# PetropoulakisPanagiotis/ICP-Variants

Hardware: AMD Instinct MI355X
Metric: ICP iterations/s (k-NN + point-to-plane linear, 370k-point ETH-Apartment-like pair) (higher is better)
Workload: dtype f32

## Files before the change

### icp-variants_amd/csrc/dev_bvh.hpp

```cpp
#ifndef ICP_ISEL_NATURAL
#define ICP_ISEL_NATURAL 0
#endif
#ifndef ICP_PRUNE_SLACK
#define ICP_PRUNE_SLACK 1.001f
#endif
constexpr int BVH_LEAF = 8;
#ifndef ICP_BVH_THREADS
#define ICP_BVH_THREADS 256
#endif
constexpr int BVH_THREADS = ICP_BVH_THREADS;
#ifndef ICP_QUERIES_PER_WAVE
#define ICP_QUERIES_PER_WAVE 64
#endif
constexpr int BVH_QPW = ICP_QUERIES_PER_WAVE;
constexpr int BVH_QPB = BVH_THREADS / 64 * BVH_QPW;
__host__ __device__ inline int fused_nblocks(int n) { return (n + BVH_QPB - 1) / BVH_QPB; }

template <int DIM> struct BvhNodeT { float lo[DIM][2]; float hi[DIM][2]; float pad[DIM == 3 ? 4 : 8]; };
template <int DIM> struct BvhLeafT { float c[DIM][BVH_LEAF]; int idx[BVH_LEAF]; float pad[DIM == 3 ? 0 : 8]; };
template <> struct BvhLeafT<3> { float c[3][BVH_LEAF]; int idx[BVH_LEAF]; };
typedef BvhNodeT<3> BvhNode;
typedef BvhLeafT<3> BvhLeaf;

template <int DIM> struct BvhQuadT { float lo[DIM][4]; float hi[DIM][4]; float pad[DIM == 3 ? 8 : 16]; };

struct TgtRec { float x, y, z; int idx; float nx, ny, nz; uint32_t rgba; };

template <int DIM> struct CoordPtrs { const float* c[DIM]; };

template <int DIM> struct BvhViewT {
    const BvhLeafT<DIM>* leaves;
    const BvhNodeT<DIM>* nodes;
    const TgtRec* recs;
    const BvhQuadT<DIM>* qnodes;
    int Lq;
    int n_valid;
    int Lp;
    CoordPtrs<DIM> tgt;
    const int* pos_of;
};

__device__ __forceinline__ unsigned long long spread21(unsigned int v) {
    unsigned long long x = v & 0x1FFFFFull;
    x = (x | (x << 32)) & 0x1F00000000FFFFull;
    x = (x | (x << 16)) & 0x1F0000FF0000FFull;
    x = (x | (x << 8)) & 0x100F00F00F00F00Full;
    x = (x | (x << 4)) & 0x10C30C30C30C30C3ull;
    x = (x | (x << 2)) & 0x1249249249249249ull;
    return x;
}
__device__ __forceinline__ unsigned int ordered_bits(float f) {
    const unsigned int u = __float_as_uint(f);
    return (u & 0x80000000u) ? ~u : (u | 0x80000000u);
}
__device__ __forceinline__ float from_ordered_bits(unsigned int u) {
    return __uint_as_float((u & 0x80000000u) ? (u & 0x7FFFFFFFu) : ~u);
}

template <int DIM> struct AxisLists { const int* L[DIM]; };
__global__ void k_axis_keys(const float* __restrict__ plane, const int* __restrict__ ids, int nv, unsigned int* __restrict__ keys) {
    const int t = blockIdx.x * blockDim.x + threadIdx.x;
    if (t < nv) keys[t] = ordered_bits(plane[ids[t]]);
}
template <int DIM>
__global__ void k_presort_axis(const CoordPtrs<DIM> cp, const AxisLists<DIM> al, int nv, int seg_shift, int n_nodes, unsigned char* __restrict__ axis_of_node) {
    const int i = blockIdx.x * blockDim.x + threadIdx.x;
    if (i >= n_nodes) return;
    const long long start = (long long)i << seg_shift;
    int axis = 0;
    if (start < nv) {
        const int end = (int)min((long long)nv, start + (1ll << seg_shift));
        float ext = -1.f;
#pragma unroll
        for (int k = 0; k < DIM; k++) {
            const float e = cp.c[k][al.L[k][end - 1]] - cp.c[k][al.L[k][(int)start]];
            if (e > ext) { ext = e; axis = k; }
        }
    }
    axis_of_node[i] = (unsigned char)axis;
}
template <int DIM>
__global__ void k_presort_side(const AxisLists<DIM> al, int nv, int seg_shift, const unsigned char* __restrict__ axis_of_node, unsigned char* __restrict__ side ) {
    const int t = blockIdx.x * blockDim.x + threadIdx.x;
    if (t >= nv) return;
    const int i = t >> seg_shift, a = axis_of_node[i];
    int j = al.L[0][t];
#pragma unroll
    for (int k = 1; k < DIM; k++) { const int jk = al.L[k][t]; j = (a == k) ? jk : j; }
    side[j] = ((t - (i << seg_shift)) >= (1 << (seg_shift - 1))) ? 1 : 0;
}
constexpr int PRS_THREADS = 256;
template <int DIM>
__global__ __launch_bounds__(PRS_THREADS) void k_presort_count(const AxisLists<DIM> al, const unsigned char* __restrict__ side, int nv, int* __restrict__ blk_cnt ) {
    __shared__ int wc[PRS_THREADS / WAVE];
    const int k = blockIdx.y, t = blockIdx.x * PRS_THREADS + threadIdx.x;
    int j = 0;
#pragma unroll
    for (int q = 0; q < DIM; q++) { if (q == k) j = t < nv ? al.L[q][t] : 0; }
    const bool f = t < nv && side[j] != 0;
    const unsigned long long m = __ballot(f);
    if ((threadIdx.x & 63) == 0) wc[threadIdx.x >> 6] = __popcll(m);
    __syncthreads();
    if (threadIdx.x == 0) blk_cnt[(size_t)k * gridDim.x + blockIdx.x] = (wc[0] + wc[1]) + (wc[2] + wc[3]);
}
__global__ __launch_bounds__(1024) void k_presort_blockscan(const int* __restrict__ blk_cnt, int nblk, int* __restrict__ blk_off ) {
    __shared__ int part[1024];
    const int* in = blk_cnt + (size_t)blockIdx.x * nblk; int* out = blk_off + (size_t)blockIdx.x * nblk;
    const int per = (nblk + 1023) / 1024, b0 = threadIdx.x * per;
    int sum = 0;
    for (int q = 0; q < per; q++) if (b0 + q < nblk) sum += in[b0 + q];
    part[threadIdx.x] = sum;
    __syncthreads();
    for (int o = 1; o < 1024; o <<= 1) {
        const int v = threadIdx.x >= o ? part[threadIdx.x - o] : 0;
        __syncthreads();
        part[threadIdx.x] += v;
        __syncthreads();
    }
    int run = part[threadIdx.x] - sum;
    for (int q = 0; q < per; q++) if (b0 + q < nblk) { out[b0 + q] = run; run += in[b0 + q]; }
}
template <int DIM>
__global__ __launch_bounds__(PRS_THREADS) void k_presort_scatter(const AxisLists<DIM> al, const unsigned char* __restrict__ side, const int* __restrict__ blk_off, int nv, int seg_shift,
                                                                 AxisLists<DIM> out_lists) {
    __shared__ int wc[PRS_THREADS / WAVE];
    const int k = blockIdx.y, t = blockIdx.x * PRS_THREADS + threadIdx.x, lane = threadIdx.x & 63, w = threadIdx.x >> 6;
    int j = 0;
#pragma unroll
    for (int q = 0; q < DIM; q++) { if (q == k) j = t < nv ? al.L[q][t] : 0; }
    const bool f = t < nv && side[j] != 0;
    const unsigned long long m = __ballot(f);
    if (lane == 0) wc[w] = __popcll(m);
    __syncthreads();
    int before = __popcll(m & ((1ull << lane) - 1ull));
    for (int ww = 0; ww < w; ww++) before += wc[ww];
    if (t >= nv) return;
    const int* off = blk_off + (size_t)k * gridDim.x;
    const int S = (t >> seg_shift) << seg_shift;
    const int r_before = off[blockIdx.x] + before - off[S / PRS_THREADS];
    const int cnt = min(1 << seg_shift, nv - S), nleft = min(1 << (seg_shift - 1), cnt);
    const int pos = f ? S + nleft + r_before : S + (t - S - r_before);
#pragma unroll
    for (int q = 0; q < DIM; q++) { if (q == k) ((int*)out_lists.L[q])[pos] = j; }
}

constexpr int BLV_POINTS = 2048, BLV_THREADS = 256, BLV_PER = BLV_POINTS / BLV_THREADS;
template <int DIM>
__global__ __launch_bounds__(BLV_THREADS) void k_bvh_block_levels(const CoordPtrs<DIM> cp, const int* __restrict__ perm_in, int n_valid, int first_shift ,
                                                                  int* __restrict__ perm_out) {
    __shared__ unsigned long long keys[BLV_POINTS];
    __shared__ int vals[BLV_POINTS];
    __shared__ unsigned int wbox[BLV_THREADS / WAVE][2 * DIM];
    const int tid = threadIdx.x, lane = tid & 63, w = tid >> 6;
    const int base = blockIdx.x * BLV_POINTS;
#pragma unroll
    for (int q = 0; q < BLV_PER; q++) { const int pos = tid * BLV_PER + q, gi = base + pos; vals[pos] = gi < n_valid ? perm_in[gi] : -1; }
    __syncthreads();
    for (int sh = first_shift; sh >= 4; sh--) {
        const int S = 1 << sh, g = S / BLV_PER;
        unsigned int lo[DIM], hi[DIM];
#pragma unroll
        for (int k = 0; k < DIM; k++) { lo[k] = 0xFFFFFFFFu; hi[k] = 0u; }
        for (int q = 0; q < BLV_PER; q++) {
            const int j = vals[tid * BLV_PER + q];
            if (j >= 0) {
#pragma unroll
                for (int k = 0; k < DIM; k++) { const unsigned int o = ordered_bits(cp.c[k][j]); lo[k] = min(lo[k], o); hi[k] = max(hi[k], o); }
            }
        }
        for (int off = 1; off < g && off < WAVE; off <<= 1) {
#pragma unroll
            for (int k = 0; k < DIM; k++) { lo[k] = min(lo[k], (unsigned int)__shfl_xor((int)lo[k], off, WAVE)); hi[k] = max(hi[k], (unsigned int)__shfl_xor((int)hi[k], off, WAVE)); }
        }
        if (g > WAVE) {
            if (lane == 0) {
#pragma unroll
                for (int k = 0; k < DIM; k++) { wbox[w][k] = lo[k]; wbox[w][DIM + k] = hi[k]; }
            }
            __syncthreads();
            const int nw = g / WAVE, w0 = w & ~(nw - 1);
            for (int ww = w0; ww < w0 + nw; ww++) {
#pragma unroll
                for (int k = 0; k < DIM; k++) { lo[k] = min(lo[k], wbox[ww][k]); hi[k] = max(hi[k], wbox[ww][DIM + k]); }
            }
        }
        int axis = 0; float ext = -1.f;
#pragma unroll
        for (int k = 0; k < DIM; k++) {
            const unsigned int uh = hi[k], ul = lo[k];
#if ICP_ISEL_NATURAL
            const float fh = from_ordered_bits(uh), fl = from_ordered_bits(ul);
#else
            const float fh = __uint_as_float((uh & 0x80000000u) ? (uh ^ 0x80000000u) : ~uh), fl = __uint_as_float((ul & 0x80000000u) ? (ul ^ 0x80000000u) : ~ul);
#endif
            const float e = fh - fl;
            if (e > ext) { ext = e; axis = k; }
        }
        for (int q = 0; q < BLV_PER; q++) {
            const int pos = tid * BLV_PER + q, j = vals[pos];
            unsigned long long key = ~0ull;
            if (j >= 0) {
#if ICP_ISEL_NATURAL
                const float c = cp.c[axis][j];
#else
                float c = cp.c[0][j];
#pragma unroll
                for (int k = 1; k < DIM; k++) c = (axis == k) ? cp.c[k][j] : c;
#endif
                key = ((unsigned long long)ordered_bits(c) << 32) | (unsigned int)pos;
            }
            keys[pos] = key;
        }
        __syncthreads();
        for (int k = 2; k <= S; k <<= 1) {
            for (int j = k >> 1; j > 0; j >>= 1) {
#pragma unroll
                for (int pp = 0; pp < BLV_POINTS / 2 / BLV_THREADS; pp++) {
                    const int idx = tid + BLV_THREADS * pp;
                    const int i = ((idx & ~(j - 1)) << 1) | (idx & (j - 1)), ip = i + j;
                    const bool asc = ((i & k) == 0) || (k == S);
                    const unsigned long long a = keys[i], b = keys[ip];
                    if ((a > b) == asc) { keys[i] = b; keys[ip] = a; const int va = vals[i]; vals[i] = vals[ip]; vals[ip] = va; }
                }
                __syncthreads();
            }
        }
    }
#pragma unroll
    for (int q = 0; q < BLV_PER; q++) { const int pos = tid * BLV_PER + q, gi = base + pos; if (gi < n_valid) perm_out[gi] = vals[pos]; }
}

template <int DIM>
__global__ void k_bvh_gather(const CoordPtrs<DIM> cp, const float* __restrict__ nx, const float* __restrict__ ny, const float* __restrict__ nz, const uint32_t* __restrict__ rgba,
                             const int* __restrict__ sorted_idx, int n_valid, int n_slots, BvhLeafT<DIM>* __restrict__ leaves, TgtRec* __restrict__ recs, int* __restrict__ pos_of) {
    const int i = blockIdx.x * blockDim.x + threadIdx.x;
    if (i >= n_slots) return;
    BvhLeafT<DIM>* lf = leaves + (i / BVH_LEAF); const int t = i % BVH_LEAF;
    TgtRec r; r.x = INFINITY; r.y = INFINITY; r.z = INFINITY; r.idx = -1; r.nx = 0.f; r.ny = 0.f; r.nz = 0.f; r.rgba = 0u;
    if (i < n_valid) {
        const int j = sorted_idx[i];
#pragma unroll
        for (int k = 0; k < DIM; k++) lf->c[k][t] = cp.c[k][j];
        lf->idx[t] = j;
        r.x = cp.c[0][j]; r.y = cp.c[1][j]; r.z = cp.c[2][j]; r.idx = j;
        if (nx) { r.nx = nx[j]; r.ny = ny[j]; r.nz = nz[j]; }
        if (rgba) r.rgba = rgba[j];
        pos_of[j] = i;
    } else {
#pragma unroll
        for (int k = 0; k < DIM; k++) lf->c[k][t] = (k < 3) ? INFINITY : 0.f;
        lf->idx[t] = -1;
    }
    recs[i] = r;
}

template <int DIM>
__device__ __forceinline__ void child_box(const BvhLeafT<DIM>* __restrict__ leaves, const BvhNodeT<DIM>* __restrict__ nodes, int child, int Lp, int n_leaves,
                                          bool child_is_leaf, float* lo, float* hi) {
#pragma unroll
    for (int k = 0; k < DIM; k++) { lo[k] = INFINITY; hi[k] = -INFINITY; }
    if (child_is_leaf) {
        const int leaf = child - (Lp - 1);
        if (leaf < n_leaves) {
            const BvhLeafT<DIM>* lf = leaves + leaf;
            for (int t = 0; t < BVH_LEAF; t++) {
                if (lf->c[0][t] < INFINITY) {
#pragma unroll
                    for (int k = 0; k < DIM; k++) { lo[k] = fminf(lo[k], lf->c[k][t]); hi[k] = fmaxf(hi[k], lf->c[k][t]); }
                }
            }
        }
    } else {
        const BvhNodeT<DIM>* nd = nodes + child;
#pragma unroll
        for (int k = 0; k < DIM; k++) { lo[k] = fminf(nd->lo[k][0], nd->lo[k][1]); hi[k] = fmaxf(nd->hi[k][0], nd->hi[k][1]); }
    }
}
template <int DIM>
__global__ void k_bvh_nodes(const BvhLeafT<DIM>* __restrict__ leaves, int n_leaves, int Lp, int first, int count, int children_are_leaves, BvhNodeT<DIM>* __restrict__ nodes) {
    const int t = blockIdx.x * blockDim.x + threadIdx.x;
    if (t >= count) return;
    const int node = first + t;
    float lo0[DIM], hi0[DIM], lo1[DIM], hi1[DIM];
    child_box<DIM>(leaves, nodes, 2 * node + 1, Lp, n_leaves, children_are_leaves != 0, lo0, hi0);
    child_box<DIM>(leaves, nodes, 2 * node + 2, Lp, n_leaves, children_are_leaves != 0, lo1, hi1);
    BvhNodeT<DIM>* out = nodes + node;
#pragma unroll
    for (int k = 0; k < DIM; k++) { out->lo[k][0] = lo0[k]; out->lo[k][1] = lo1[k]; out->hi[k][0] = hi0[k]; out->hi[k][1] = hi1[k]; }
}

template <int DIM>
__global__ void k_bvh_quad_nodes(const BvhNodeT<DIM>* __restrict__ nodes, int pad, int Lq, BvhQuadT<DIM>* __restrict__ qnodes) {
    const int t = blockIdx.x * blockDim.x + threadIdx.x;
    const int total = (int)((((1ll << (2 * Lq)) - 1) / 3) * 4);
    if (t >= total) return;
    const int q = t >> 2, c = t & 3;
    int l = 0; while ((int)(((1ll << (2 * (l + 1))) - 1) / 3) <= q) l++;
    const int idx = q - (int)(((1ll << (2 * l)) - 1) / 3);
    const int rd = 2 * l + 2 - pad, ri = 4 * idx + c;
    float lo[DIM], hi[DIM];
#pragma unroll
    for (int k = 0; k < DIM; k++) { lo[k] = INFINITY; hi[k] = -INFINITY; }
    if (ri < (1 << rd)) {
        const BvhNodeT<DIM>* nd = nodes + ((1 << (rd - 1)) - 1 + (ri >> 1));
#pragma unroll
        for (int k = 0; k < DIM; k++) { lo[k] = nd->lo[k][ri & 1]; hi[k] = nd->hi[k][ri & 1]; }
    }
#pragma unroll
    for (int k = 0; k < DIM; k++) { qnodes[q].lo[k][c] = lo[k]; qnodes[q].hi[k][c] = hi[k]; }
}

template <int DIM>
__device__ __forceinline__ f2 pair_lb(const BvhNodeT<DIM>* __restrict__ nd, const f2* p2) {
    f2 acc;
#pragma unroll
    for (int k = 0; k < DIM; k++) {
        const f2 lo = *(const f2*)nd->lo[k], hi = *(const f2*)nd->hi[k];
        const f2 a = lo - p2[k], b = p2[k] - hi;
        const f2 e = {fmaxf(fmaxf(a.x, b.x), 0.f), fmaxf(fmaxf(a.y, b.y), 0.f)};
        const f2 sq = e * e;
        acc = (k == 0) ? sq : acc + sq;
    }
    return acc;
}

__device__ __forceinline__ float sqrt_up(float x) { return __builtin_amdgcn_sqrtf(fmaxf(x, 1.17549435e-38f)) * 1.000001f; }
__device__ __forceinline__ float sqrt_dn(float x) { return __builtin_amdgcn_sqrtf(x) * 0.999999f; }

__device__ __forceinline__ void others_insert(float x, int xl, float& b2, int& l2, float& b3) {
    const bool better = x < b2, same = xl == l2;
    b3 = same ? b3 : fminf(b3, better ? b2 : x);
    l2 = better ? xl : l2; b2 = better ? x : b2;
}

template <int DIM>
__device__ __forceinline__ void leaf_eval(const BvhLeafT<DIM>* __restrict__ lf, int leaf, const f2* p2, float& best, int& bi, int& bpos, float& b2, int& l2, float& b3) {
    const int prev_leaf = bpos >> 3; const float prev_best = best;
    float dd[BVH_LEAF];
    float m = FLT_MAX;
#pragma unroll
    for (int t = 0; t < BVH_LEAF; t += 2) {
        f2 d;
#pragma unroll
        for (int k = 0; k < DIM; k++) {
            const f2 q = *(const f2*)(&lf->c[k][t]);
            const f2 e = p2[k] - q;
            const f2 sq = e * e;
            d = (k == 0) ? sq : d + sq;
        }
        dd[t] = d.x; dd[t + 1] = d.y;
        m = fminf(fminf(m, d.x), d.y);
    }
    if (m <= best) {
        float mo = FLT_MAX;
        bool here = prev_leaf == leaf;
#pragma unroll
        for (int t = 0; t < BVH_LEAF; t++) {
            const int j = lf->idx[t];
            const bool take = (dd[t] < best) | ((dd[t] == best) & (j < bi));
            const float other = take ? (here ? best : FLT_MAX) : ((j != bi) ? dd[t] : FLT_MAX);
            mo = fminf(mo, other);
            here = here | take;
            best = take ? dd[t] : best; bi = take ? j : bi; bpos = take ? leaf * BVH_LEAF + t : bpos;
        }
        others_insert(mo, leaf, b2, l2, b3);
        if (prev_leaf != leaf && (bpos >> 3) == leaf) others_insert(prev_best, prev_leaf, b2, l2, b3);
    } else others_insert(m, leaf, b2, l2, b3);
}

template <int DIM>
__device__ __forceinline__ void seed_from_previous(const int* __restrict__ nn_pos, int use_prev, const BvhViewT<DIM>& bv, int k, const float* p, float& best, int& bi, int& bpos) {
    if (!use_prev) return;
    const int q0 = nn_pos[k];
    if (q0 < 0) return;
    float t[DIM]; int j0;
    if (DIM == 3) { const float4 r = *(const float4*)(bv.recs + q0); t[0] = r.x; t[1] = r.y; t[2] = r.z; j0 = __float_as_int(r.w); }
    else {
        const BvhLeafT<DIM>* lf = bv.leaves + (q0 >> 3);
#pragma unroll
        for (int q = 0; q < DIM; q++) t[q] = lf->c[q][q0 & 7];
        j0 = lf->idx[q0 & 7];
    }
    float d = 0.f;
#pragma unroll
    for (int q = 0; q < DIM; q++) { const float e = p[q] - t[q]; d = (q == 0) ? e * e : d + e * e; }
    if (d < best) { best = d; bi = j0; bpos = q0; }
}

struct TravState { int depth; int idx; unsigned int pending; bool alive; };

__device__ __forceinline__ void trav_pop(TravState& st, const unsigned short* __restrict__ lb16, int tid, int nthreads, float best, float& minlb) {
    while (!st.alive && st.pending) {
        const int d = 31 - __clz((int)st.pending);
        st.pending &= ~(1u << d);
        const float lb = __uint_as_float((unsigned int)lb16[d * nthreads + tid] << 16);
        if (!(lb * 0.99999f > best)) { st.idx = (st.idx >> (st.depth - d - 1)) ^ 1; st.depth = d + 1; st.alive = true; }
        else minlb = fminf(minlb, lb);
    }
}

template <class MaskT> struct QuadStateT { int L; int idx; MaskT pending; bool alive; };

template <int DIM>
__device__ __forceinline__ void quad_lb(const BvhQuadT<DIM>* __restrict__ nd, const f2* p2, f2& l01, f2& l23) {
#pragma unroll
    for (int k = 0; k < DIM; k++) {
        const f2 lo0 = *(const f2*)&nd->lo[k][0], lo1 = *(const f2*)&nd->lo[k][2], hi0 = *(const f2*)&nd->hi[k][0], hi1 = *(const f2*)&nd->hi[k][2];
        const f2 a0 = lo0 - p2[k], b0 = p2[k] - hi0, a1 = lo1 - p2[k], b1 = p2[k] - hi1;
        const f2 e0 = {fmaxf(fmaxf(a0.x, b0.x), 0.f), fmaxf(fmaxf(a0.y, b0.y), 0.f)};
        const f2 e1 = {fmaxf(fmaxf(a1.x, b1.x), 0.f), fmaxf(fmaxf(a1.y, b1.y), 0.f)};
        const f2 s0 = e0 * e0, s1 = e1 * e1;
        l01 = (k == 0) ? s0 : l01 + s0;
        l23 = (k == 0) ? s1 : l23 + s1;
    }
}

template <int DIM> struct QueryPt { f2 p2[DIM]; };
template <int DIM>
__device__ __forceinline__ void make_query(const BvhViewT<DIM>& bv, const float* p, QueryPt<DIM>& q) {
#pragma unroll
    for (int k = 0; k < DIM; k++) { q.p2[k].x = p[k]; q.p2[k].y = p[k]; }
}
template <int DIM>
__device__ __forceinline__ void quad_lb_at(const BvhViewT<DIM>& bv, unsigned int node, const QueryPt<DIM>& q, f2& l01, f2& l23) {
    quad_lb<DIM>(bv.qnodes + node, q.p2, l01, l23);
}

template <class MaskT>
__device__ __forceinline__ void quad_pop_bits(QuadStateT<MaskT>& st) {
    if (!st.alive && st.pending) {
        const int top = sizeof(MaskT) == 8 ? 63 - __clzll((long long)st.pending) : 31 - __clz((int)st.pending);
        const int lv = top >> 2;
        const unsigned int bits = (unsigned int)(st.pending >> (4 * lv)) & 0xFu;
        const int c = __ffs((int)bits) - 1;
        st.pending &= ~((MaskT)1 << (4 * lv + c));
        st.idx = ((st.idx >> (2 * (st.L - lv))) << 2) | c; st.L = lv + 1; st.alive = true;
    }
}
#ifndef ICP_DEBUG_STEPS
#define ICP_DEBUG_STEPS 0
#endif

__device__ __forceinline__ int xcd_contiguous_block(int b, int nb) {
    constexpr int C = 16;
    const int full = nb / (8 * C) * (8 * C);
    if (b >= full) return b;
    const int x = b & 7, j = b >> 3;
    return ((j / C) * 8 + x) * C + j % C;
}

template <int DIM>
__device__ __forceinline__ void knn_load_query(const KnnParams& kp, int k, float* p) {
    const int i = kp.sel ? kp.sel[k] : k;
    p[0] = kp.sx[i]; p[1] = kp.sy[i]; p[2] = kp.sz[i];
    if (!kp.pretransformed) { float a, b, c; xform_point(kp.ps->pose, p[0], p[1], p[2], a, b, c); p[0] = a; p[1] = b; p[2] = c; }
    if (DIM == 6) { p[3 % DIM] = kp.scr[i]; p[4 % DIM] = kp.scg[i]; p[5 % DIM] = kp.scb[i]; }
}

template <int DIM>
__device__ __forceinline__ bool knn_try_verify(const KnnParams& kp, const BvhViewT<DIM>& bv, int k, const float* p, float& best, int& bi, int& bpos, float& lb_others) {
    seed_from_previous<DIM>(kp.nn_raw, kp.use_prev, bv, k, p, best, bi, bpos);
    if (kp.incremental && kp.use_prev && bi >= 0) {
        const float4 s = kp.qstate[k];
        const float ex = p[0] - s.x, ey = p[1] - s.y, ez = p[2] - s.z;
        const float delta = sqrt_up((ex * ex + ey * ey) + ez * ez);
        const float lbn = (s.w - delta) * 0.999999f;
        if (sqrt_up(best) < lbn) { lb_others = lbn; return true; }
    }
    return false;
}

template <int DIM>
__device__ __forceinline__ void knn_store_state(const KnnParams& kp, int k, const float* p, float best, int bpos, float lb_others, float lb3, int l2) {
    if (kp.qstate) { float4 s; s.x = p[0]; s.y = p[1]; s.z = p[2]; s.w = lb_others; kp.qstate[k] = s; }
    if (kp.qstate2) { float2 t; t.x = lb3; t.y = __int_as_float(l2); kp.qstate2[k] = t; }
    if (kp.nn_raw) kp.nn_raw[k] = bpos;
    if (kp.d2_out) kp.d2_out[k] = best;
}

#ifndef ICP_SHARE_ROUNDS
#define ICP_SHARE_ROUNDS 2
#endif
#define ICP_SHARE_ROWS 10
#ifndef ICP_XW_SLEEP
#define ICP_XW_SLEEP 4
#endif
constexpr int XW_SLOTS = 64, XW_CTRL = 64;
#if defined(ICP_DEBUG_TIMES) && ICP_DEBUG_TIMES
__device__ unsigned int g_dev_counts[16];
#define DEV_COUNT(i, n) atomicAdd(&g_dev_counts[i], (unsigned int)(n))
#ifndef ICP_DEBUG_WALK_TRACE
#define ICP_DEBUG_WALK_TRACE 0
#endif
__device__ unsigned int g_walk_trace[64];
#else
#define DEV_COUNT(i, n)
#endif
constexpr int XW_INTS = XW_CTRL + XW_SLOTS + XW_SLOTS * 5;
constexpr int XW_SPIN_LIMIT = 1 << 22;
template <int DIM, int NT> constexpr bool xw_enabled() { return DIM == 3 && NT > WAVE && NT / WAVE <= 8; }
template <int DIM, int NT> constexpr size_t xw_lds_bytes() { return xw_enabled<DIM, NT>() ? (size_t)XW_INTS * 4 : 0; }
template <int NT> __device__ __forceinline__ void xw_init(uint2* lbq, int tid) { if (tid < XW_CTRL + XW_SLOTS) ((int*)(lbq + ICP_SHARE_ROWS * NT))[tid] = 0; }
template <int NT> __device__ __forceinline__ bool xw_block_is_searching(uint2* lbq) {
    const int* xc = (const int*)(lbq + ICP_SHARE_ROWS * NT);
    const int nreg = __builtin_amdgcn_readfirstlane(__hip_atomic_load(xc + 0, __ATOMIC_RELAXED, __HIP_MEMORY_SCOPE_WORKGROUP)), ndone = __builtin_amdgcn_readfirstlane(__hip_atomic_load(xc + 1, __ATOMIC_RELAXED, __HIP_MEMORY_SCOPE_WORKGROUP));
    return nreg > ndone;
}

template <int DIM, int NT, class MaskT, int MODE = 0>
__device__ __forceinline__ void knn_walk_shared(const BvhViewT<DIM>& bv, float* p, float* keep3, bool need_walk, float& best, int& bi, int& bpos, float& lb_others, float& lb3, int& l2o,
                                                uint2* __restrict__ lbq, int tid, int* fault = nullptr) {
    constexpr bool XW = MODE == 1 || MODE == 2, HELP = MODE == 2;
    static_assert(!XW || xw_enabled<DIM, NT>(), "cross-wave sharing: DIM 3, 2..8 waves per block");
    const int lane = tid & 63, Lq = bv.Lq, wbase = tid & ~63, myw = tid >> 6;
    uint2* R = lbq + wbase;
    constexpr unsigned int FMAXB = 0x7F7FFFFFu, NONE = 0x7F800000u;
    unsigned long long* keys = (unsigned long long*)lbq;
    int* xc = (int*)(lbq + ICP_SHARE_ROWS * NT);
    int* xstate = xc + XW_CTRL; uint2* xa = (uint2*)(xstate + XW_SLOTS); uint2* xb = xa + XW_SLOTS; int* xp = (int*)(xb + XW_SLOTS);
    if (!HELP) {
        R[3 * NT + lane] = make_uint2(__float_as_uint(best), (unsigned int)bi);
        R[4 * NT + lane] = make_uint2((unsigned int)bpos, __float_as_uint(lb_others));
        R[5 * NT + lane] = make_uint2(__float_as_uint(lb3), __float_as_uint(p[0]));
        R[7 * NT + lane] = make_uint2(__float_as_uint(p[1]), __float_as_uint(p[2]));
        R[8 * NT + lane] = make_uint2(__float_as_uint(keep3[0]), __float_as_uint(keep3[1]));
        R[9 * NT + lane] = make_uint2(__float_as_uint(keep3[2]), (unsigned int)l2o);
        keys[tid] = ~0ull;
        keys[NT + tid] = ~0ull;
        R[2 * NT + lane] = make_uint2(FMAXB, 0xFFFFFFFFu);
        ((unsigned int*)(R + 6 * NT))[WAVE + lane] = FMAXB;
    }
    auto fold_part = [&](int owner, float wb, int wi, int wp, float b2, int l2, float b3, unsigned int mlb) {
        const unsigned long long mykey = ((unsigned long long)__float_as_uint(wb) << 32) | (unsigned int)wi;
        const unsigned long long old = __hip_atomic_fetch_min(keys + owner, mykey, __ATOMIC_RELAXED, __HIP_MEMORY_SCOPE_WORKGROUP);
        unsigned int* bp = (unsigned int*)(lbq + 2 * NT + owner);
        unsigned int rest = __float_as_uint(b3);
        unsigned long long e = ((unsigned long long)__float_as_uint(b2) << 32) | (unsigned int)l2;
        if (old < mykey) {
            const unsigned long long w = ((unsigned long long)__float_as_uint(wb) << 32) | (unsigned int)(wp >> 3);
            const unsigned long long lo = w < e ? w : e, hi = w < e ? e : w;
            if ((unsigned int)lo != (unsigned int)hi) rest = min(rest, (unsigned int)(hi >> 32));
            e = lo;
        } else if (old > mykey && old != ~0ull) rest = min(rest, (unsigned int)(old >> 32));
        {
            const unsigned long long o2 = __hip_atomic_fetch_min(keys + NT + owner, e, __ATOMIC_RELAXED, __HIP_MEMORY_SCOPE_WORKGROUP);
            const unsigned long long lo = o2 < e ? o2 : e, hi = o2 < e ? e : o2;
            if (hi != ~0ull && (unsigned int)lo != (unsigned int)hi) rest = min(rest, (unsigned int)(hi >> 32));
        }
        __hip_atomic_fetch_min(bp, rest, __ATOMIC_RELAXED, __HIP_MEMORY_SCOPE_WORKGROUP);
        __hip_atomic_fetch_min((unsigned int*)(lbq + 6 * NT + (owner & ~63)) + WAVE + (owner & 63), mlb, __ATOMIC_RELAXED, __HIP_MEMORY_SCOPE_WORKGROUP);
        if (__hip_atomic_load(keys + owner, __ATOMIC_RELAXED, __HIP_MEMORY_SCOPE_WORKGROUP) == mykey) bp[1] = (unsigned int)wp;
    };
    bool lone_done = false;
    const unsigned long long wm0 = __ballot(need_walk);
    if (MODE == 1 && DIM == 3 && sizeof(MaskT) == 4 && Lq > 0 && __popcll(wm0) == 1 && wm0 == __ballot(need_walk && bpos >= 0)) {
        int* tbl = (int*)(R + 6 * NT);
        const int wl = (int)__ffsll((long long)wm0) - 1;
        QueryPt<DIM> lq;
#pragma unroll
        for (int a = 0; a < DIM; a++) { const float v = __shfl(p[a], wl, WAVE); lq.p2[a].x = v; lq.p2[a].y = v; }
        const float sb = __shfl(best, wl, WAVE); const int si = __shfl(bi, wl, WAVE), sp = __shfl(bpos, wl, WAVE);
        const float thr_u = fminf(sb * ICP_PRUNE_SLACK, FLT_MAX);
        unsigned int lmlb = FMAXB;
        int nf = 1, L = 0; bool ok = true;
        if (lane == 0) tbl[0] = 0;
        while (L < Lq && ok) {
            const int items = nf * 4;
            const bool act = lane < items;
            const int n = act ? tbl[lane >> 2] : 0, j = lane & 3;
            f2 a01, a23;
            quad_lb_at<DIM>(bv, (0x55555555u & ((1u << (2 * L)) - 1u)) + (unsigned int)n, lq, a01, a23);
            const float lbj = j == 0 ? a01.x : j == 1 ? a01.y : j == 2 ? a23.x : a23.y;
            const bool alive = act && !(lbj > thr_u);
            if (act && !alive) lmlb = min(lmlb, __float_as_uint(lbj));
            const int c = 4 * n + j;
            if (L + 2 <= Lq) {
                f2 g01, g23;
                quad_lb_at<DIM>(bv, (0x55555555u & ((1u << (2 * (L + 1))) - 1u)) + (unsigned int)(act ? c : 0), lq, g01, g23);
                const bool s0 = alive && !(g01.x > thr_u), s1 = alive && !(g01.y > thr_u), s2 = alive && !(g23.x > thr_u), s3 = alive && !(g23.y > thr_u);
                if (alive) lmlb = min(min(lmlb, min(s0 ? NONE : __float_as_uint(g01.x), s1 ? NONE : __float_as_uint(g01.y))), min(s2 ? NONE : __float_as_uint(g23.x), s3 ? NONE : __float_as_uint(g23.y)));
                const unsigned long long m0 = __ballot(s0), m1 = __ballot(s1), m2 = __ballot(s2), m3 = __ballot(s3);
                const int c0 = __popcll(m0), c1 = __popcll(m1), c2 = __popcll(m2), nn = c0 + c1 + c2 + __popcll(m3);
                ok = nn <= (L + 2 < Lq ? 16 : WAVE);
                if (ok) {
                    const unsigned long long below = (1ull << lane) - 1ull;
                    if (s0) tbl[__popcll(m0 & below)] = 4 * c;
                    if (s1) tbl[c0 + __popcll(m1 & below)] = 4 * c + 1;
                    if (s2) tbl[c0 + c1 + __popcll(m2 & below)] = 4 * c + 2;
                    if (s3) tbl[c0 + c1 + c2 + __popcll(m3 & below)] = 4 * c + 3;
                }
                nf = nn; L += 2;
            } else {
                const unsigned long long m = __ballot(alive);
                if (alive) tbl[__popcll(m & ((1ull << lane) - 1ull))] = c;
                nf = __popcll(m); L += 1;
            }
        }
        if (ok) {
            if (lane < nf) {
                const int leaf = tbl[lane];
                float xb = sb, x2 = FLT_MAX, x3 = FLT_MAX; int xi = si, xp = sp, xl = -1;
                leaf_eval<DIM>(bv.leaves + leaf, leaf, lq.p2, xb, xi, xp, x2, xl, x3);
                fold_part(wbase + wl, xb, xi, xp, x2, xl, x3, lmlb);
            } else __hip_atomic_fetch_min((unsigned int*)(lbq + 6 * NT + wbase) + WAVE + wl, lmlb, __ATOMIC_RELAXED, __HIP_MEMORY_SCOPE_WORKGROUP);
            lone_done = true;
        }
#if ICP_DEBUG_TIMES
        if (lane == 0) DEV_COUNT(ok ? 11 : 12, 1);
#endif
    }
    QueryPt<DIM> qp;
    float wb; int wi, wp;
    if constexpr (DIM == 3 && MODE == 1 && sizeof(MaskT) == 4) {
        const uint2 ra_ = R[3 * NT + lane], rb_ = R[4 * NT + lane], rc_ = R[5 * NT + lane], rd_ = R[7 * NT + lane];
        float pq[3] = {__uint_as_float(rc_.y), __uint_as_float(rd_.x), __uint_as_float(rd_.y)};
        make_query<DIM>(bv, pq, qp);
        wb = __uint_as_float(ra_.x); wi = (int)ra_.y; wp = (int)rb_.x;
    } else {
        make_query<DIM>(bv, p, qp);
        wb = best; wi = bi; wp = bpos;
    }
    if (!HELP && need_walk && !lone_done) {
        if (wp < 0) {
            int idx = 0;
            for (int L = 0; L < Lq; L++) {
                f2 l01, l23;
                quad_lb_at<DIM>(bv, (0x55555555u & ((1u << (2 * L)) - 1u)) + (unsigned int)idx, qp, l01, l23);
                const float m = fminf(fminf(l01.x, l01.y), fminf(l23.x, l23.y));
                const int c = (l01.x == m) ? 0 : (l01.y == m) ? 1 : (l23.x == m) ? 2 : 3;
                idx = (idx << 2) | c;
            }
            float u2 = FLT_MAX, u3 = FLT_MAX; int ul = -1;
            leaf_eval<DIM>(bv.leaves + idx, idx, qp.p2, wb, wi, wp, u2, ul, u3);
        }
    }
    const unsigned long long wm = __ballot(need_walk);
    const int W = __popcll(wm);
#if ICP_DEBUG_TIMES && ICP_DEBUG_WALK_TRACE
    const bool tracer = !HELP && W > 0 && W <= 3 && lane == (int)__ffsll((long long)wm) - 1;
    if (tracer) { g_walk_trace[0] = (unsigned int)W; g_walk_trace[2] = (unsigned int)wall_clock64(); }
#endif
    if (MODE == 1 && lane == 0 && !lone_done) __hip_atomic_fetch_add(xc + 0, 1, __ATOMIC_RELAXED, __HIP_MEMORY_SCOPE_WORKGROUP);
    const bool spread = !HELP && Lq > 0 && W > 0 && W * (Lq + 1) <= WAVE && wm == __ballot(need_walk && wp >= 0);
    float b2 = FLT_MAX, b3 = FLT_MAX; int l2 = -1;
    unsigned int mlb = FMAXB;
    int owner = need_walk ? tid : -1;
    QuadStateT<MaskT> st; st.L = 0; st.idx = 0; st.pending = 0; st.alive = need_walk;
    float thr = fminf(wb * ICP_PRUNE_SLACK, FLT_MAX);
    auto descend = [&](const f2& l01, const f2& l23) {
        const float m = fminf(fminf(l01.x, l01.y), fminf(l23.x, l23.y));
        const bool s0 = !(l01.x > thr), s1 = !(l01.y > thr), s2 = !(l23.x > thr), s3 = !(l23.y > thr);
        mlb = min(min(mlb, min(s0 ? NONE : __float_as_uint(l01.x), s1 ? NONE : __float_as_uint(l01.y))), min(s2 ? NONE : __float_as_uint(l23.x), s3 ? NONE : __float_as_uint(l23.y)));
        if (!(m > thr)) {
            const bool c0 = l01.x == m, c1 = l01.y == m, c2 = l23.x == m;
            int c = 3; c = c2 ? 2 : c; c = c1 ? 1 : c; c = c0 ? 0 : c;
            const unsigned int pend = ((s0 ? 1u : 0u) | (s1 ? 2u : 0u) | (s2 ? 4u : 0u) | (s3 ? 8u : 0u)) & ~(1u << c);
            st.pending |= (MaskT)pend << (4 * st.L);
            st.idx = (st.idx << 2) | c; st.L++;
        } else st.alive = false;
        quad_pop_bits(st);
    };
    if (spread && !lone_done) {
        int* tbl = (int*)(R + 6 * NT);
        if (need_walk) tbl[__builtin_amdgcn_mbcnt_hi((unsigned int)(wm >> 32), __builtin_amdgcn_mbcnt_lo((unsigned int)wm, 0u))] = lane;
        const bool two = W * (2 * Lq + 2) <= WAVE;
        const int roles = two ? 2 * Lq + 1 : Lq;
#if ICP_DEBUG_TIMES && ICP_DEBUG_WALK_TRACE
        if (tracer) g_walk_trace[1] = two ? 2u : 1u;
#endif
        const unsigned long long im = ~wm;
        const int ri = (int)__builtin_amdgcn_mbcnt_hi((unsigned int)(im >> 32), __builtin_amdgcn_mbcnt_lo((unsigned int)im, 0u));
        const int r = (ri * ((65536 + roles - 1) / roles)) >> 16, role = ri - r * roles;
        bool take = !need_walk && r < W;
        const int src = take ? tbl[r] : lane;
        float q[DIM];
#pragma unroll
        for (int a = 0; a < DIM; a++) q[a] = __shfl(qp.p2[a].x, src, WAVE);
        const float sb = __shfl(wb, src, WAVE); const int si = __shfl(wi, src, WAVE), sp = __shfl(wp, src, WAVE);
        const int sl2 = two ? __shfl(l2o, src, WAVE) : -1;
        const int leafA = sp >> 3;
        const bool onB = role >= Lq;
        const int L = role == 2 * Lq ? Lq : (onB ? role - Lq : role);
        const int myleaf = onB ? sl2 : leafA;
        const int nodeA = leafA >> (2 * (Lq - L)), nodeB = sl2 >> (2 * (Lq - L));
        if (onB && (sl2 < 0 || nodeB == nodeA)) take = false;
        if (take) {
#pragma unroll
            for (int a = 0; a < DIM; a++) { qp.p2[a].x = q[a]; qp.p2[a].y = q[a]; }
            wb = sb; wi = si; wp = sp; owner = wbase + src;
            thr = fminf(wb * ICP_PRUNE_SLACK, FLT_MAX);
            st.L = L; st.idx = myleaf >> (2 * (Lq - L)); st.alive = true;
            if (L < Lq) {
                const int skip = (myleaf >> (2 * (Lq - L - 1))) & 3;
                const int skipB = (!onB && sl2 >= 0 && nodeB == nodeA) ? (sl2 >> (2 * (Lq - L - 1))) & 3 : skip;
                f2 l01, l23;
                quad_lb_at<DIM>(bv, (0x55555555u & ((1u << (2 * L)) - 1u)) + (unsigned int)st.idx, qp, l01, l23);
                const float inf = __uint_as_float(NONE);
                l01.x = (skip == 0 || skipB == 0) ? inf : l01.x; l01.y = (skip == 1 || skipB == 1) ? inf : l01.y;
                l23.x = (skip == 2 || skipB == 2) ? inf : l23.x; l23.y = (skip == 3 || skipB == 3) ? inf : l23.y;
                descend(l01, l23);
            }
        }
        if (need_walk) { st.L = Lq; st.idx = wp >> 3; }
    }
#if ICP_DEBUG_TIMES && ICP_DEBUG_WALK_TRACE
    if (tracer) g_walk_trace[3] = (unsigned int)wall_clock64();
#endif
    bool polling = false;
    int polls = 0;
#if ICP_DEBUG_TIMES && ICP_DEBUG_WALK_TRACE
    int trips = 0;
#endif
    for (; !lone_done;) {
#if ICP_DEBUG_TIMES && ICP_DEBUG_WALK_TRACE
        trips++;
        if (tracer && trips < 56) g_walk_trace[7 + trips] = (unsigned int)wall_clock64();
#endif
        if (!st.alive && owner >= 0) {
            fold_part(owner, wb, wi, wp, b2, l2, b3, mlb);
            if (XW && (owner >> 6) != myw) __hip_atomic_fetch_sub(xc + 4 + (owner >> 6), 1, __ATOMIC_RELEASE, __HIP_MEMORY_SCOPE_WORKGROUP);
            owner = -1;
        }
        if (!__any(st.alive)) {
            if (!XW) break;
            const bool complete = MODE == 1 && __builtin_amdgcn_readfirstlane(__hip_atomic_load(xc + 4 + myw, __ATOMIC_ACQUIRE, __HIP_MEMORY_SCOPE_WORKGROUP)) == 0;
            const int sv = complete ? 0 : __hip_atomic_load(xstate + lane, __ATOMIC_RELAXED, __HIP_MEMORY_SCOPE_WORKGROUP);
            bool mine = false;
            if (sv == 1) { int expect = 1; mine = __hip_atomic_compare_exchange_strong(xstate + lane, &expect, 3, __ATOMIC_ACQUIRE, __ATOMIC_RELAXED, __HIP_MEMORY_SCOPE_WORKGROUP); }
            if (mine) {
                const uint2 ia = xa[lane], ib = xb[lane]; const int ip = xp[lane];
                __hip_atomic_store(xstate + lane, 0, __ATOMIC_RELEASE, __HIP_MEMORY_SCOPE_WORKGROUP);
                owner = (int)(ia.x & 0xFFFFu);
                if ((owner >> 6) == myw) __hip_atomic_fetch_sub(xc + 4 + myw, 1, __ATOMIC_RELAXED, __HIP_MEMORY_SCOPE_WORKGROUP);
                const uint2 c = lbq[5 * NT + owner], d = lbq[7 * NT + owner];
                qp.p2[0].x = __uint_as_float(c.y); qp.p2[0].y = qp.p2[0].x; qp.p2[1].x = __uint_as_float(d.x); qp.p2[1].y = qp.p2[1].x; qp.p2[2 % DIM].x = __uint_as_float(d.y); qp.p2[2 % DIM].y = qp.p2[2 % DIM].x;
                wb = __uint_as_float(ib.x); wi = (int)ib.y; wp = ip;
                b2 = FLT_MAX; b3 = FLT_MAX; l2 = -1; mlb = FMAXB;
                thr = fminf(wb * ICP_PRUNE_SLACK, FLT_MAX);
                st.L = (int)(ia.x >> 16); st.idx = (int)ia.y; st.pending = 0; st.alive = true;
            }
            if (__any(mine)) {
                if (polling) { polling = false; if (lane == 0) __hip_atomic_fetch_sub(xc + 2, 1, __ATOMIC_RELAXED, __HIP_MEMORY_SCOPE_WORKGROUP); }
            } else {
                if (MODE == 1) {
                    if (complete) { if (lane == 0) __hip_atomic_fetch_add(xc + 1, 1, __ATOMIC_RELAXED, __HIP_MEMORY_SCOPE_WORKGROUP); break; }
                } else {
                    const int ndone = __builtin_amdgcn_readfirstlane(__hip_atomic_load(xc + 1, __ATOMIC_RELAXED, __HIP_MEMORY_SCOPE_WORKGROUP)), nreg = __builtin_amdgcn_readfirstlane(__hip_atomic_load(xc + 0, __ATOMIC_RELAXED, __HIP_MEMORY_SCOPE_WORKGROUP));
                    if (ndone >= nreg) break;
                }
                if (!polling) { polling = true; if (lane == 0) __hip_atomic_fetch_add(xc + 2, 1, __ATOMIC_RELAXED, __HIP_MEMORY_SCOPE_WORKGROUP); }
                if (++polls > XW_SPIN_LIMIT) { if (fault && lane == 0) atomicOr(fault, 1); break; }
                __builtin_amdgcn_s_sleep(ICP_XW_SLEEP);
                continue;
            }
        }
        bool served = true;
#pragma unroll 1
        for (int round = 0; round < ICP_SHARE_ROUNDS; round++) {
            const unsigned long long im = __ballot(owner < 0);
            if (!im) break;
            const bool can = st.alive && st.pending != 0;
            const unsigned long long dm = __ballot(can);
            served = __popcll(im) <= __popcll(dm);
            if (!dm) break;
            {
                const int n = min(__popcll(im), __popcll(dm));
                int* tbl = (int*)(R + 6 * NT);
                int dL = 0, dIdx = 0;
                const int rd = (int)__builtin_amdgcn_mbcnt_hi((unsigned int)(dm >> 32), __builtin_amdgcn_mbcnt_lo((unsigned int)dm, 0u));
                if (can && rd < n) {
                    const int low = sizeof(MaskT) == 8 ? __ffsll((long long)st.pending) - 1 : __ffs((int)st.pending) - 1;
                    const int lv = low >> 2;
                    st.pending &= ~((MaskT)1 << low);
                    dL = lv + 1; dIdx = ((st.idx >> (2 * (st.L - lv))) << 2) | (low & 3);
                    tbl[rd] = lane;
                }
                const int ri = (int)__builtin_amdgcn_mbcnt_hi((unsigned int)(im >> 32), __builtin_amdgcn_mbcnt_lo((unsigned int)im, 0u));
                const bool take = owner < 0 && ri < n;
                const int src = take ? tbl[ri] : lane;
                float q[DIM];
#pragma unroll
                for (int a = 0; a < DIM; a++) q[a] = __shfl(qp.p2[a].x, src, WAVE);
                const float sb = __shfl(wb, src, WAVE); const int si = __shfl(wi, src, WAVE), sp = __shfl(wp, src, WAVE), so = __shfl(owner, src, WAVE);
                const int sL = __shfl(dL, src, WAVE), sI = __shfl(dIdx, src, WAVE);
                if (take) {
#pragma unroll
                    for (int a = 0; a < DIM; a++) { qp.p2[a].x = q[a]; qp.p2[a].y = q[a]; }
                    wb = sb; wi = si; wp = sp; owner = so;
                    b2 = FLT_MAX; b3 = FLT_MAX; l2 = -1; mlb = FMAXB;
                    thr = fminf(wb * ICP_PRUNE_SLACK, FLT_MAX);
                    st.L = sL; st.idx = sI; st.pending = 0; st.alive = true;
                    if (XW && (so >> 6) != myw) __hip_atomic_fetch_add(xc + 4 + (so >> 6), 1, __ATOMIC_RELAXED, __HIP_MEMORY_SCOPE_WORKGROUP);
                }
            }
        }
        const int idlew = (XW && served) ? __builtin_amdgcn_readfirstlane(__hip_atomic_load(xc + 2, __ATOMIC_RELAXED, __HIP_MEMORY_SCOPE_WORKGROUP)) : 0;
        if (XW && served && idlew > 0) {
            const bool can = st.alive && st.pending != 0;
            const unsigned long long dm = __ballot(can);
            if (dm) {
                const int sv = __hip_atomic_load(xstate + lane, __ATOMIC_RELAXED, __HIP_MEMORY_SCOPE_WORKGROUP);
                const unsigned long long fm = __ballot(sv == 0);
                const int n = min(__popcll(dm), __popcll(fm));
                int* tbl = (int*)(R + 6 * NT);
                const int rf = (int)__builtin_amdgcn_mbcnt_hi((unsigned int)(fm >> 32), __builtin_amdgcn_mbcnt_lo((unsigned int)fm, 0u));
                if (sv == 0 && rf < n) tbl[rf] = lane;
                const int rd = (int)__builtin_amdgcn_mbcnt_hi((unsigned int)(dm >> 32), __builtin_amdgcn_mbcnt_lo((unsigned int)dm, 0u));
                if (can && rd < n) {
                    const int slot = tbl[rd];
                    int expect = 0;
                    if (__hip_atomic_compare_exchange_strong(xstate + slot, &expect, 2, __ATOMIC_RELAXED, __ATOMIC_RELAXED, __HIP_MEMORY_SCOPE_WORKGROUP)) {
                        const int low = sizeof(MaskT) == 8 ? __ffsll((long long)st.pending) - 1 : __ffs((int)st.pending) - 1;
                        const int lv = low >> 2;
                        st.pending &= ~((MaskT)1 << low);
                        xa[slot] = make_uint2((unsigned int)owner | ((unsigned int)(lv + 1) << 16), (unsigned int)(((st.idx >> (2 * (st.L - lv))) << 2) | (low & 3)));
                        xb[slot] = make_uint2(__float_as_uint(wb), (unsigned int)wi);
                        xp[slot] = wp;
                        __hip_atomic_fetch_add(xc + 4 + (owner >> 6), 1, __ATOMIC_RELAXED, __HIP_MEMORY_SCOPE_WORKGROUP);
                        __hip_atomic_store(xc + 12 + (owner >> 6), 1, __ATOMIC_RELAXED, __HIP_MEMORY_SCOPE_WORKGROUP);
                        __hip_atomic_store(xstate + slot, 1, __ATOMIC_RELEASE, __HIP_MEMORY_SCOPE_WORKGROUP);
                    }
                }
            }
        }
        while (st.alive && st.L < Lq) {
            f2 l01, l23;
            quad_lb_at<DIM>(bv, (0x55555555u & ((1u << (2 * st.L)) - 1u)) + (unsigned int)st.idx, qp, l01, l23);
            descend(l01, l23);
            if (served ? __any(!st.alive) : __any(st.pending != 0)) break;
        }
        if (st.alive && st.L == Lq) {
            leaf_eval<DIM>(bv.leaves + st.idx, st.idx, qp.p2, wb, wi, wp, b2, l2, b3);
            thr = fminf(wb * ICP_PRUNE_SLACK, FLT_MAX);
            st.alive = false;
            quad_pop_bits(st);
        }
    }
    if (XW && polling && lane == 0) __hip_atomic_fetch_sub(xc + 2, 1, __ATOMIC_RELAXED, __HIP_MEMORY_SCOPE_WORKGROUP);
#if ICP_DEBUG_TIMES && ICP_DEBUG_WALK_TRACE
    if (tracer) { g_walk_trace[4] = (unsigned int)trips; g_walk_trace[5] = (unsigned int)polls; g_walk_trace[6] = (unsigned int)wall_clock64(); }
#endif
    asm volatile("" ::"v"(0u));
    if (HELP) return;
    {
        const uint2 c = R[5 * NT + lane], d = R[7 * NT + lane], e = R[8 * NT + lane], f = R[9 * NT + lane];
        p[0] = __uint_as_float(c.y); p[1] = __uint_as_float(d.x); p[2] = __uint_as_float(d.y);
        keep3[0] = __uint_as_float(e.x); keep3[1] = __uint_as_float(e.y); keep3[2] = __uint_as_float(f.x);
    }
    if (need_walk) {
        const unsigned long long key = keys[tid], key2 = keys[NT + tid];
        const uint2 b = R[2 * NT + lane];
        best = __uint_as_float((unsigned int)(key >> 32)); bi = (int)(unsigned int)key; bpos = (int)b.y;
        const float sk = __uint_as_float(((const unsigned int*)(R + 6 * NT))[WAVE + lane]);
        const float rest = fminf(__uint_as_float(b.x), sk);
        lb_others = sqrt_dn(fminf(__uint_as_float((unsigned int)(key2 >> 32)), rest));
        lb3 = sqrt_dn(rest);
        l2o = key2 == ~0ull ? -1 : (int)(unsigned int)key2;
        if (XW && __builtin_amdgcn_readfirstlane(__hip_atomic_load(xc + 12 + myw, __ATOMIC_RELAXED, __HIP_MEMORY_SCOPE_WORKGROUP))) {
            if (bi < 0) { bpos = -1; DEV_COUNT(13, 1); }
            else if (bpos < 0 || bv.recs[bpos].idx != bi) bpos = bv.pos_of[bi];
        }
    } else {
        const uint2 a = R[3 * NT + lane], b = R[4 * NT + lane], c = R[5 * NT + lane];
        best = __uint_as_float(a.x); bi = (int)a.y; bpos = (int)b.x; lb_others = __uint_as_float(b.y); lb3 = __uint_as_float(c.x); l2o = (int)R[9 * NT + lane].y;
    }
}


template <int DIM, int NT, class MaskT>
__device__ __forceinline__ void xw_help(const BvhViewT<DIM>& bv, uint2* __restrict__ lbq, int tid, int* fault) {
    float p[DIM], k3[3] = {0.f, 0.f, 0.f}, best = FLT_MAX, lbo = 0.f, lb3 = 0.f; int bi = -1, bpos = -1, l2 = -1;
#pragma unroll
    for (int q = 0; q < DIM; q++) p[q] = 0.f;
    knn_walk_shared<DIM, NT, MaskT, 2>(bv, p, k3, false, best, bi, bpos, lbo, lb3, l2, lbq, tid, fault);
}

template <int DIM>
__device__ __forceinline__ void knn_bvh_query(const KnnParams& kp, const BvhViewT<DIM>& bv, int k, uint2* __restrict__ lbq, int tid,
                                              float& best, int& bi, int& bpos) {
    float p[DIM];
#pragma unroll
    for (int q = 0; q < DIM; q++) p[q] = 0.f;
    if (k >= 0) knn_load_query<DIM>(kp, k, p);
    best = FLT_MAX; bi = -1; bpos = -1;
    float lb_others = 0.f, lb3 = 0.f; int l2 = -1;
    bool need_walk = false;
    if (k >= 0 && finite3(p[0], p[1], p[2]) && bv.n_valid > 0) {
        if (knn_try_verify<DIM>(kp, bv, k, p, best, bi, bpos, lb_others)) lb3 = lb_others;
        else need_walk = true;
    }
    if (__any(need_walk)) {
        float none[3] = {0.f, 0.f, 0.f};
        if (bv.Lq <= 8) knn_walk_shared<DIM, BVH_THREADS, unsigned int>(bv, p, none, need_walk, best, bi, bpos, lb_others, lb3, l2, lbq, tid);
        else knn_walk_shared<DIM, BVH_THREADS, unsigned long long>(bv, p, none, need_walk, best, bi, bpos, lb_others, lb3, l2, lbq, tid);
    }
    if (k >= 0) knn_store_state<DIM>(kp, k, p, best, bpos, lb_others, lb3, l2);
}

__device__ __forceinline__ int knn_bvh_lane_query(const KnnParams& kp, const int* __restrict__ qorder, int tid) {
    const int t = xcd_contiguous_block(blockIdx.x, gridDim.x) * BVH_THREADS + tid;
    if (t >= kp.n) return -1;
    return qorder ? qorder[t] : t;
}

template <int DIM>
__global__ __launch_bounds__(BVH_THREADS) void k_knn_bvh(const KnnParams kp, const BvhViewT<DIM> bv, const int* __restrict__ qorder) {
#include "dev_body_knn_bvh.hpp"
}
```

### icp-variants_amd/csrc/dev_fused.hpp

```cpp
struct RowSlotGen {
    const RowTerms& R;
    static constexpr int N = 27;
    template <int A> __device__ __forceinline__ double get() const { return row_slot<A>(R); }
};
struct P2pGen {
    float s[3], d[3]; double wd;
    static constexpr int N = 22;
    template <int A> __device__ __forceinline__ double get() const {
        double v;
        if constexpr (A < 3) v = (double)s[A];
        else if constexpr (A < 6) v = (double)d[A - 3];
        else if constexpr (A == 6) v = wd;
        else if constexpr (A < 10) v = wd * s[A - 7];
        else if constexpr (A < 13) v = wd * d[A - 10];
        else v = (double)d[(A - 13) / 3] * (wd * s[(A - 13) % 3]);
        return v;
    }
};
#ifndef ICP_FUSED_WAVES
#define ICP_FUSED_WAVES 6
#endif
#ifndef ICP_WAVE_STRIDE
#define ICP_WAVE_STRIDE (ICP_BVH_THREADS > 64 ? 128 : 0)
#endif
#ifndef ICP_DEBUG_WALK_ENDS
#define ICP_DEBUG_WALK_ENDS 0
#endif
#ifndef ICP_DEBUG_TIMES
#define ICP_DEBUG_TIMES 0
#endif
#if ICP_DEBUG_TIMES
#define ICP_STAMP(j) do { if (kp.dbg_steps && lane == 0) kp.dbg_steps[8 * (wave_slot) + (j)] = (int)(unsigned int)wall_clock64(); } while (0)
#else
#define ICP_STAMP(j)
#endif

template <int DIM> struct QueryIn {
    float r0, r1, r2;
    float c3, c4, c5;
    float rn0, rn1, rn2;
    int q0;
    float4 st;
    float4 ra, rb;
    float tq[DIM]; int j0;
};
template <int DIM>
__device__ __forceinline__ void fused_front_clear(QueryIn<DIM>& in) {
    in.r0 = 0.f; in.r1 = 0.f; in.r2 = 0.f; in.c3 = 0.f; in.c4 = 0.f; in.c5 = 0.f; in.rn0 = 0.f; in.rn1 = 0.f; in.rn2 = 0.f; in.q0 = -1; in.j0 = -1;
    in.st.x = 0.f; in.st.y = 0.f; in.st.z = 0.f; in.st.w = 0.f; in.ra = in.st; in.rb = in.st;
#pragma unroll
    for (int q = 0; q < DIM; q++) in.tq[q] = 0.f;
}
template <int DIM>
__device__ __forceinline__ void fused_front_loads(const KnnParams& kp, const PostParams& pp, const BvhViewT<DIM>& bv, int k, bool seeded, bool inc, QueryIn<DIM>& in) {
    fused_front_clear<DIM>(in);
    if (k >= 0) {
        const int i = kp.sel ? kp.sel[k] : k;
        in.r0 = kp.sx[i]; in.r1 = kp.sy[i]; in.r2 = kp.sz[i];
        if (DIM == 6) { in.c3 = kp.scr[i]; in.c4 = kp.scg[i]; in.c5 = kp.scb[i]; }
        in.rn0 = pp.snx[i]; in.rn1 = pp.sny[i]; in.rn2 = pp.snz[i];
        in.q0 = seeded ? kp.nn_raw[k] : -1;
        if (inc) in.st = kp.qstate[k];
        if (in.q0 >= 0) {
            if (DIM == 3) { in.ra = *(const float4*)(bv.recs + in.q0); in.rb = *((const float4*)(bv.recs + in.q0) + 1); in.tq[0] = in.ra.x; in.tq[1] = in.ra.y; in.tq[2] = in.ra.z; in.j0 = __float_as_int(in.ra.w); }
            else {
                const BvhLeafT<DIM>* lf = bv.leaves + (in.q0 >> 3);
#pragma unroll
                for (int q = 0; q < DIM; q++) in.tq[q] = lf->c[q][in.q0 & 7];
                in.j0 = lf->idx[in.q0 & 7];
            }
        }
    }
}

__host__ __device__ __forceinline__ int fused_wave_slot(int lb, int w, int mgrid) {
    constexpr int NW = BVH_THREADS / WAVE, S = ICP_WAVE_STRIDE;
    if (S == 0 || NW == 1) return lb * NW + w;
    if (S == 1) return w * mgrid + lb;
    const int g = lb / S, j = lb - g * S;
    return (g + 1) * S <= mgrid ? (g * NW + w) * S + j : lb * NW + w;
}

struct PairOut { bool valid; float s0, s1, s2, d0, d1, d2, n0, n1, n2, wt; };

template <int DIM, bool WIDE, bool XW = false>
__device__ __forceinline__ void fused_search_post(const KnnParams& kp, const BvhViewT<DIM>& bv, const PostParams& pp, int k, bool seeded, bool inc, const float* Pm, const float* Nm,
                                                  QueryIn<DIM>& in, uint2* __restrict__ bvh_lbq, int tid, int wave_slot, PairOut& o) {
    const int lane = tid & 63; (void)lane; (void)wave_slot; (void)seeded;
    o.valid = false; o.s0 = 0.f; o.s1 = 0.f; o.s2 = 0.f; o.d0 = 0.f; o.d1 = 0.f; o.d2 = 0.f; o.n0 = 0.f; o.n1 = 0.f; o.n2 = 0.f; o.wt = 0.f;
    float p[DIM];
#pragma unroll
    for (int q = 0; q < DIM; q++) p[q] = 0.f;
    if (DIM == 6) { p[3 % DIM] = in.c3; p[4 % DIM] = in.c4; p[5 % DIM] = in.c5; }
    float rn0 = in.rn0, rn1 = in.rn1, rn2 = in.rn2;
    float best = FLT_MAX, lb_others = 0.f; int bi = -1, bpos = -1, q0 = in.q0;
    float4 ra = in.ra, rb = in.rb;
#if ICP_DEBUG_TIMES
    float dbg_lbo = 0.f, dbg_lb3 = 0.f, dbg_delta = 0.f; int dbg_l2old = -1; const int dbg_q0old = in.q0;
#endif
    bool need_walk = false, verified = false, two_leaf = false;
    float lb3 = 0.f; int l2 = -1;
    if (k >= 0) {
        float2 st2; st2.x = 0.f; st2.y = __int_as_float(-1);
        xform_point(Pm, in.r0, in.r1, in.r2, p[0], p[1], p[2]);
        if (finite3(p[0], p[1], p[2]) && bv.n_valid > 0) {
            need_walk = true;
            if (q0 >= 0) {
                float d = 0.f;
#pragma unroll
                for (int q = 0; q < DIM; q++) { const float e = p[q] - in.tq[q]; d = (q == 0) ? e * e : d + e * e; }
                if (d < best) { best = d; bi = in.j0; bpos = q0; }
                if (inc && bi >= 0) {
                    const float ex = p[0] - in.st.x, ey = p[1] - in.st.y, ez = p[2] - in.st.z;
                    const float delta = sqrt_up((ex * ex + ey * ey) + ez * ez), sbest = sqrt_up(best);
                    const float lbn = (in.st.w - delta) * 0.999999f;
#if ICP_DEBUG_TIMES
                    dbg_lbo = in.st.w; dbg_lb3 = st2.x; dbg_delta = delta;
#endif
                    if (sbest < lbn) { lb_others = lbn; need_walk = false; verified = true; }
                    else {
                        if (kp.qstate2) st2 = kp.qstate2[k];
#if ICP_DEBUG_TIMES
                        dbg_l2old = __float_as_int(st2.y);
#endif
                        const float lb2 = (st2.x - delta) * 0.999999f;
                        l2 = __float_as_int(st2.y);
                        if (sbest < lb2) { two_leaf = true; lb3 = lb2; }
                    }
                }
            }
        }
    }
    ICP_STAMP(1);
#if ICP_DEBUG_TIMES
    if (kp.dbg_steps && k >= 0 && (need_walk || two_leaf) && seeded) {
        int* r = kp.dbg_steps + 8 * kp.dbg_waves + 8 * (k & 4095);
        r[0] = k; r[1] = __float_as_int(best); r[2] = __float_as_int(dbg_lbo); r[3] = __float_as_int(dbg_lb3); r[4] = __float_as_int(dbg_delta); r[5] = two_leaf ? l2 : -2; r[6] = q0; r[7] = (int)(unsigned int)wall_clock64();
    }
    if (kp.dbg_steps) { const int nw_ = __popcll(__ballot(need_walk && !two_leaf)), nl_ = __popcll(__ballot(two_leaf)); if (lane == 0) { kp.dbg_steps[8 * wave_slot + 6] = nw_ | (nl_ << 8);
            kp.dbg_steps[8 * wave_slot + 7] = (int)((__builtin_amdgcn_s_getreg((31 << 11) | 4) & 0xFFFFu) | (__builtin_amdgcn_s_getreg((31 << 11) | 20) << 16)); } }
#endif
    if (two_leaf) {
        f2 p2[DIM];
#pragma unroll
        for (int q = 0; q < DIM; q++) { p2[q].x = p[q]; p2[q].y = p[q]; }
        float b2 = FLT_MAX, b3 = FLT_MAX; int nl2 = -1;
        const int lf = q0 >> 3;
        leaf_eval<DIM>(bv.leaves + lf, lf, p2, best, bi, bpos, b2, nl2, b3);
        if (l2 >= 0 && l2 != lf) leaf_eval<DIM>(bv.leaves + l2, l2, p2, best, bi, bpos, b2, nl2, b3);
        lb_others = fminf(sqrt_dn(b2), lb3);
        lb3 = fminf(sqrt_dn(b3), lb3);
        l2 = nl2;
        need_walk = false;
    }
#if ICP_DEBUG_STEPS && !ICP_DEBUG_TIMES
    if (k >= 0 && kp.dbg_steps) kp.dbg_steps[k] = need_walk ? -1 : two_leaf ? -2 : 0;
#endif
    bool walked = false;
    if (__any(need_walk)) {
        walked = true;
        float rn[3] = {rn0, rn1, rn2};
        knn_walk_shared<DIM, BVH_THREADS, typename std::conditional<WIDE, unsigned long long, unsigned int>::type, XW ? 1 : 0>(bv, p, rn, need_walk, best, bi, bpos, lb_others, lb3, l2, bvh_lbq, tid, kp.fault);
        rn0 = rn[0]; rn1 = rn[1]; rn2 = rn[2];
        q0 = -2;
        fused_front_clear<DIM>(in);
    }
    ICP_STAMP(2);
#if ICP_DEBUG_TIMES && ICP_DEBUG_WALK_ENDS
    if (k >= 0 && need_walk && seeded) {
        DEV_COUNT(8, 1);
        if (dbg_q0old >= 0 && (bpos >> 3) == (dbg_q0old >> 3)) DEV_COUNT(9, 1);
        if (dbg_l2old >= 0 && (bpos >> 3) == dbg_l2old) DEV_COUNT(10, 1);
    }
#endif
    asm volatile("" : "+v"(k));
    if (k >= 0) {
        if (!verified) knn_store_state<DIM>(kp, k, p, best, bpos, lb_others, lb3, l2);
        else if (kp.d2_out) kp.d2_out[k] = best;
        icp_match_t m;
        if (best <= kp.max_dist) { m.idx = bi; m.weight = 1.f; } else { m.idx = -1; m.weight = 0.f; }
        if (m.idx < 0) { if (pp.matches) pp.matches[k] = m; }
        else {
            if (walked || DIM != 3 || bpos != q0) { ra = *(const float4*)(bv.recs + bpos); rb = *((const float4*)(bv.recs + bpos) + 1); }
            o.d0 = ra.x; o.d1 = ra.y; o.d2 = ra.z; o.n0 = rb.x; o.n1 = rb.y; o.n2 = rb.z;
            o.s0 = p[0]; o.s1 = p[1]; o.s2 = p[2];
            o.valid = post_eval<true>(pp, k, m, o.d0, o.d1, o.d2, o.n0, o.n1, o.n2, __float_as_uint(rb.w), o.s0, o.s1, o.s2, o.wt, rn0, rn1, rn2, Nm);
        }
    }
    ICP_STAMP(3);
}

template <class StoreFn>
__device__ __forceinline__ void fused_block_epilogue(const KnnParams& kp, const PostParams& pp, PairOut& o, uint2* __restrict__ bvh_lbq, int tid, int wave_slot, const StoreFn& store) {
    constexpr int NW = BVH_THREADS / WAVE;
    const int lane = tid & 63, w = tid >> 6; (void)wave_slot; (void)kp;
    __syncthreads();
    double* lds = (double*)bvh_lbq;
    double tot;
    if (!o.valid) { o.s0 = 0.f; o.s1 = 0.f; o.s2 = 0.f; o.d0 = 0.f; o.d1 = 0.f; o.d2 = 0.f; o.n0 = 0.f; o.n1 = 0.f; o.n2 = 0.f; o.wt = 0.f; }
    if (pp.metric == ICP_METRIC_POINT_TO_PLANE) {
        RowTerms R;
        build_rows(0, o.s0, o.s1, o.s2, o.d0, o.d1, o.d2, o.n0, o.n1, o.n2, o.wt, R);
        const RowSlotGen g{R};
        tot = wave_transpose_reduce_gen<6, 0>(g, lane);
    } else {
        const P2pGen g{{o.s0, o.s1, o.s2}, {o.d0, o.d1, o.d2}, (double)o.wt};
        tot = wave_transpose_reduce_gen<6, 0>(g, lane);
    }
    ICP_STAMP(4);
    {
        const unsigned long long vm = __ballot(o.valid);
        const int v = wave_value_of_lane(lane);
        if (v < 32) lds[w * 32 + v] = tot;
        if (lane == 0) lds[NW * 32 + w] = (double)__popcll(vm);
    }
    __syncthreads();
    if (tid < NSUM_USED) {
        double out = 0.0;
        if (tid == SUM_N) { for (int ww = 0; ww < NW; ww++) out += lds[NW * 32 + ww]; }
        else {
            const int v = pp.metric == ICP_METRIC_POINT_TO_PLANE ? tid - SUM_M : tid - 1;
            const int nv = pp.metric == ICP_METRIC_POINT_TO_PLANE ? 27 : 22;
            if (v >= 0 && v < nv) { for (int ww = 0; ww < NW; ww++) out += lds[ww * 32 + v]; }
        }
        store(tid, out);
    }
    ICP_STAMP(5);
}

template <int DIM, bool WIDE, bool MERGED>
__device__ __forceinline__ void fused_matcher_body(const KnnParams& kp, const BvhViewT<DIM>& bv, const int* __restrict__ qorder, const PostParams& pp, const RingParams& rp) {
    extern __shared__ uint2 bvh_lbq[];
    constexpr int NW = BVH_THREADS / WAVE;
    if constexpr (MERGED) { if ((int)blockIdx.x < rp.n_red) { if (BVH_THREADS == RING_THREADS || threadIdx.x < RING_THREADS) ring_reduce_solve(rp); return; } }
    const int n_red = MERGED ? rp.n_red : 0;
    const int mblock = (int)blockIdx.x - n_red, mgrid = (int)gridDim.x - n_red;
    typedef const __attribute__((address_space(4))) float* cfloat_p;
    float Pm[16], Nm[9];
    if constexpr (!MERGED) {
        const cfloat_p pc = (cfloat_p)(const void*)kp.ps->pose; const cfloat_p nc = (cfloat_p)(const void*)kp.ps->nmat;
#pragma unroll
        for (int q = 0; q < 16; q++) Pm[q] = pc[q];
#pragma unroll
        for (int q = 0; q < 9; q++) Nm[q] = nc[q];
    }
    const int tid = threadIdx.x, lane = tid & 63, w = tid >> 6;
    const int lb = xcd_contiguous_block(mblock, mgrid);
    const int wave_slot = fused_wave_slot(lb, w, mgrid);
    const int t = wave_slot * BVH_QPW + lane;
    ICP_STAMP(0);
    const int k = ((BVH_QPW == WAVE || lane < BVH_QPW) && t < kp.n) ? (qorder ? qorder[t] : t) : -1;
    const bool seeded = kp.use_prev != 0, inc = kp.incremental && seeded;
    QueryIn<DIM> in;
    fused_front_loads<DIM>(kp, pp, bv, k, seeded, inc, in);
    constexpr bool XW = xw_enabled<DIM, BVH_THREADS>();
    if constexpr (XW) {
        xw_init<BVH_THREADS>(bvh_lbq, tid);
        asm volatile("s_waitcnt lgkmcnt(0)\n\ts_barrier" ::: "memory");
    }
    if constexpr (MERGED) { if (!ring_wait_pose(loop_slot((PoseState*)kp.ps, 0, (int)((blockIdx.x * 2u + (unsigned int)w) % (unsigned int)POSE_REPLICAS)), lane, rp.run_fault, Pm, Nm)) return; }
    PairOut o;
    fused_search_post<DIM, WIDE, XW>(kp, bv, pp, k, seeded, inc, Pm, Nm, in, bvh_lbq, tid, wave_slot, o);
    if constexpr (XW) {
        if (xw_block_is_searching<BVH_THREADS>(bvh_lbq)) {
            constexpr int NT = BVH_THREADS;
            bvh_lbq[3 * NT + tid] = make_uint2(__float_as_uint(o.s0), __float_as_uint(o.s1)); bvh_lbq[4 * NT + tid] = make_uint2(__float_as_uint(o.s2), __float_as_uint(o.d0));
            bvh_lbq[5 * NT + tid] = make_uint2(__float_as_uint(o.d1), __float_as_uint(o.d2)); bvh_lbq[7 * NT + tid] = make_uint2(__float_as_uint(o.n0), __float_as_uint(o.n1));
            bvh_lbq[8 * NT + tid] = make_uint2(__float_as_uint(o.n2), __float_as_uint(o.wt)); bvh_lbq[9 * NT + tid] = make_uint2(o.valid ? 1u : 0u, 0u);
            xw_help<DIM, NT, typename std::conditional<WIDE, unsigned long long, unsigned int>::type>(bv, bvh_lbq, tid, kp.fault);
            const uint2 a = bvh_lbq[3 * NT + tid], b = bvh_lbq[4 * NT + tid], c = bvh_lbq[5 * NT + tid], d = bvh_lbq[7 * NT + tid], e = bvh_lbq[8 * NT + tid], f = bvh_lbq[9 * NT + tid];
            o.s0 = __uint_as_float(a.x); o.s1 = __uint_as_float(a.y); o.s2 = __uint_as_float(b.x); o.d0 = __uint_as_float(b.y); o.d1 = __uint_as_float(c.x); o.d2 = __uint_as_float(c.y);
            o.n0 = __uint_as_float(d.x); o.n1 = __uint_as_float(d.y); o.n2 = __uint_as_float(e.x); o.wt = __uint_as_float(e.y); o.valid = f.x != 0u;
        }
    }
    double* partials = pp.partials;
    fused_block_epilogue(kp, pp, o, bvh_lbq, tid, wave_slot, [=](int a, double v) { partials[(size_t)a * mgrid + lb] = v; });
}
template <int DIM, bool WIDE>
__global__ __launch_bounds__(BVH_THREADS, DIM == 3 ? ICP_FUSED_WAVES : 4) void k_knn_bvh_post(const KnnParams kp, const BvhViewT<DIM> bv, const int* __restrict__ qorder, const PostParams pp) {
    const RingParams none{};
    fused_matcher_body<DIM, WIDE, false>(kp, bv, qorder, pp, none);
}
template <int DIM, bool WIDE>
__global__ __launch_bounds__(BVH_THREADS, DIM == 3 ? ICP_FUSED_WAVES : 4) void k_knn_bvh_post_ring(const KnnParams kp, const BvhViewT<DIM> bv, const int* __restrict__ qorder, const PostParams pp, const RingParams rp) {
    static_assert(BVH_THREADS >= RING_THREADS, "the reducer blocks are the first RING_THREADS threads of a matcher-sized block");
    fused_matcher_body<DIM, WIDE, true>(kp, bv, qorder, pp, rp);
}
```

### icp-variants_amd/csrc/host_debug.hpp

```cpp
extern "C" {
int icp_debug_steps(icp_ctx* c, int32_t* out, int32_t n) {
    if (!c || !out || n <= 0 || !c->dbg_steps.p || (size_t)n * 4 > c->dbg_steps.cap) return ICP_ERR_INVALID_ARG;
    int rc;
    if ((rc = set_device(c))) return rc;
    HIPCK(c, hipMemcpy(out, c->dbg_steps.p, (size_t)n * 4, hipMemcpyDeviceToHost));
    return ICP_OK;
}

int icp_debug_ring_times(icp_ctx* c, int32_t* out, int32_t n) {
#if ICP_DEBUG_TIMES
    if (!c || !out || n < (NSUM_USED + 1) * 8) return ICP_ERR_INVALID_ARG;
    int rc;
    if ((rc = set_device(c))) return rc;
    HIPCK(c, hipMemcpyFromSymbol(out, HIP_SYMBOL(icpdev::g_ring_dbg), (size_t)(NSUM_USED + 1) * 8 * 4));
    return ICP_OK;
#else
    (void)c; (void)out; (void)n;
    return ICP_ERR_INVALID_ARG;
#endif
}
int icp_debug_dev_counters(icp_ctx* c, uint32_t* out16, int32_t reset) {
#if ICP_DEBUG_TIMES
    if (!c || !out16) return ICP_ERR_INVALID_ARG;
    int rc;
    if ((rc = set_device(c))) return rc;
    HIPCK(c, hipStreamSynchronize(c->stream));
    HIPCK(c, hipMemcpyFromSymbol(out16, HIP_SYMBOL(icpdev::g_dev_counts), 64));
    if (reset == 2) HIPCK(c, hipMemcpyFromSymbol(out16, HIP_SYMBOL(icpdev::g_walk_trace), 256));
    if (reset) { uint32_t z[16] = {0}; HIPCK(c, hipMemcpyToSymbol(HIP_SYMBOL(icpdev::g_dev_counts), z, 64)); }
    return ICP_OK;
#else
    (void)c; (void)out16; (void)reset;
    return ICP_ERR_INVALID_ARG;
#endif
}
int icp_debug_wave_slot(int32_t lb, int32_t w, int32_t mgrid, int32_t* waves_per_block) {
    if (waves_per_block) *waves_per_block = BVH_THREADS / WAVE;
    if (lb < 0 || lb >= mgrid || w < 0 || w >= BVH_THREADS / WAVE) return -1;
    return icpdev::fused_wave_slot(lb, w, mgrid);
}
__global__ void k_debug_pos_of(const icpdev::TgtRec* recs, const int* pos_of, int n_slots, int* bad) {
    const int i = blockIdx.x * blockDim.x + threadIdx.x;
    if (i < n_slots && recs[i].idx >= 0 && pos_of[recs[i].idx] != i) atomicAdd(bad, 1);
}
int icp_debug_pos_of_mismatches(icp_ctx* c, int32_t* n_bad, int32_t* n_checked) {
    if (!c || !n_bad || !c->bvh.valid) return ICP_ERR_INVALID_ARG;
    int rc;
    if ((rc = set_device(c))) return rc;
    const int n_slots = (c->bvh.n_leaves > 0 ? c->bvh.n_leaves : 1) * BVH_LEAF;
    if ((rc = ensure(c, c->d_count, 4))) return rc;
    HIPCK(c, hipMemsetAsync(c->d_count.p, 0, 4, c->stream));
    hipLaunchKernelGGL(k_debug_pos_of, dim3((n_slots + 255) / 256), dim3(256), 0, c->stream, c->bvh.recs.as<icpdev::TgtRec>(), c->bvh.pos_of.as<int>(), n_slots, c->d_count.as<int>());
    HIPCK(c, hipMemcpyAsync(n_bad, c->d_count.p, 4, hipMemcpyDeviceToHost, c->stream));
    HIPCK(c, hipStreamSynchronize(c->stream));
    if (n_checked) *n_checked = c->bvh.n_valid;
    return ICP_OK;
}
int icp_debug_live_bytes(int64_t* out) {
    if (!out) return ICP_ERR_INVALID_ARG;
    *out = (int64_t)g_live_bytes.load();
    return ICP_OK;
}
int icp_debug_counters(icp_ctx* c, int32_t* merged_runs, int32_t* merged_fallbacks) {
    if (!c) return ICP_ERR_INVALID_ARG;
    if (merged_runs) *merged_runs = c->merged_runs;
    if (merged_fallbacks) *merged_fallbacks = c->merged_fallbacks;
    return ICP_OK;
}
int icp_debug_poison_handover(icp_ctx* c, int32_t slot, double value) {
    if (!c || slot < 0 || slot >= NSUM) return ICP_ERR_INVALID_ARG;
    int rc;
    if ((rc = set_device(c))) return rc;
    if (!c->totals.p && (rc = rearm_handover(c))) return rc;
    HIPCK(c, hipMemcpyAsync(c->totals.as<double>() + slot, &value, 8, hipMemcpyHostToDevice, c->stream));
    HIPCK(c, hipStreamSynchronize(c->stream));
    return ICP_OK;
}

int icp_selftest_wave_reduce(icp_ctx* c, const double* in, double* out, int32_t* lane_of) {
    if (!c || !in || !out || !lane_of) return ICP_ERR_INVALID_ARG;
    int rc;
    if ((rc = set_device(c))) return rc;
    DrainOnError guard(c);
    if ((rc = ensure(c, c->staging, 64 * 27 * 8 + 27 * 8 + 27 * 4 + 64))) return rc;
    double* d_in = c->staging.as<double>(); double* d_out = d_in + 64 * 27; int* d_lane = (int*)(d_out + 27);
    HIPCK(c, hipMemcpyAsync(d_in, in, 64 * 27 * 8, hipMemcpyHostToDevice, c->stream));
    hipLaunchKernelGGL(k_selftest_wave_reduce, dim3(1), dim3(64), 0, c->stream, d_in, d_out, d_lane);
    HIPCK(c, hipGetLastError());
    HIPCK(c, hipMemcpyAsync(out, d_out, 27 * 8, hipMemcpyDeviceToHost, c->stream));
    HIPCK(c, hipMemcpyAsync(lane_of, d_lane, 27 * 4, hipMemcpyDeviceToHost, c->stream));
    HIPCK(c, hipStreamSynchronize(c->stream));
    return guard.done();
}
}
```

Baseline: 34000.

## Fast-path leaf evaluation with min/second-min via med3 and clamp-based quad bounds

```diff
diff --git a/icp-variants_amd/csrc/dev_bvh.hpp b/icp-variants_amd/csrc/dev_bvh.hpp
--- a/icp-variants_amd/csrc/dev_bvh.hpp
+++ b/icp-variants_amd/csrc/dev_bvh.hpp
@@ -289,6 +289,7 @@
     for (int k = 0; k < DIM; k++) { out->lo[k][0] = lo0[k]; out->lo[k][1] = lo1[k]; out->hi[k][0] = hi0[k]; out->hi[k][1] = hi1[k]; }
 }
 
+constexpr float BVH_QUAD_EMPTY_LO = INFINITY, BVH_QUAD_EMPTY_HI = INFINITY;
 template <int DIM>
 __global__ void k_bvh_quad_nodes(const BvhNodeT<DIM>* __restrict__ nodes, int pad, int Lq, BvhQuadT<DIM>* __restrict__ qnodes) {
     const int t = blockIdx.x * blockDim.x + threadIdx.x;
@@ -306,6 +307,10 @@
 #pragma unroll
         for (int k = 0; k < DIM; k++) { lo[k] = nd->lo[k][ri & 1]; hi[k] = nd->hi[k][ri & 1]; }
     }
+    if (lo[0] > hi[0]) {
+#pragma unroll
+        for (int k = 0; k < DIM; k++) { lo[k] = BVH_QUAD_EMPTY_LO; hi[k] = BVH_QUAD_EMPTY_HI; }
+    }
 #pragma unroll
     for (int k = 0; k < DIM; k++) { qnodes[q].lo[k][c] = lo[k]; qnodes[q].hi[k][c] = hi[k]; }
 }
@@ -329,15 +334,12 @@
 
 __device__ __forceinline__ void others_insert(float x, int xl, float& b2, int& l2, float& b3) {
     const bool better = x < b2, same = xl == l2;
-    b3 = same ? b3 : fminf(b3, better ? b2 : x);
+    b3 = same ? b3 : __uint_as_float(min(__float_as_uint(b3), __float_as_uint(better ? b2 : x)));
     l2 = better ? xl : l2; b2 = better ? x : b2;
 }
 
 template <int DIM>
-__device__ __forceinline__ void leaf_eval(const BvhLeafT<DIM>* __restrict__ lf, int leaf, const f2* p2, float& best, int& bi, int& bpos, float& b2, int& l2, float& b3) {
-    const int prev_leaf = bpos >> 3; const float prev_best = best;
-    float dd[BVH_LEAF];
-    float m = FLT_MAX;
+__device__ __forceinline__ void leaf_distances(const BvhLeafT<DIM>* __restrict__ lf, const f2* p2, float* dd) {
 #pragma unroll
     for (int t = 0; t < BVH_LEAF; t += 2) {
         f2 d;
@@ -349,23 +351,71 @@
             d = (k == 0) ? sq : d + sq;
         }
         dd[t] = d.x; dd[t + 1] = d.y;
-        m = fminf(fminf(m, d.x), d.y);
-    }
-    if (m <= best) {
-        float mo = FLT_MAX;
-        bool here = prev_leaf == leaf;
-#pragma unroll
-        for (int t = 0; t < BVH_LEAF; t++) {
-            const int j = lf->idx[t];
-            const bool take = (dd[t] < best) | ((dd[t] == best) & (j < bi));
-            const float other = take ? (here ? best : FLT_MAX) : ((j != bi) ? dd[t] : FLT_MAX);
+    }
+}
+template <int DIM>
+__device__ __forceinline__ void leaf_update_sequential(const BvhLeafT<DIM>* __restrict__ lf, int leaf, const f2* p2, bool here, float& best, int& bi, int& bpos, float& mo) {
+    mo = FLT_MAX;
+#pragma unroll
+    for (int t = 0; t < BVH_LEAF; t += 2) {
+        asm volatile("" : "+v"(mo), "+v"(best), "+v"(lf));
+        f2 d;
+#pragma unroll
+        for (int k = 0; k < DIM; k++) {
+            const f2 q = *(const f2*)(&lf->c[k][t]);
+            const f2 e = p2[k] - q;
+            const f2 sq = e * e;
+            d = (k == 0) ? sq : d + sq;
+        }
+#pragma unroll
+        for (int u = 0; u < 2; u++) {
+            const float du = u ? d.y : d.x;
+            const int j = lf->idx[t + u];
+            const bool take = (du < best) | ((du == best) & (j < bi));
+            const float other = take ? (here ? best : FLT_MAX) : ((j != bi) ? du : FLT_MAX);
             mo = fminf(mo, other);
             here = here | take;
-            best = take ? dd[t] : best; bi = take ? j : bi; bpos = take ? leaf * BVH_LEAF + t : bpos;
-        }
-        others_insert(mo, leaf, b2, l2, b3);
-        if (prev_leaf != leaf && (bpos >> 3) == leaf) others_insert(prev_best, prev_leaf, b2, l2, b3);
-    } else others_insert(m, leaf, b2, l2, b3);
+            best = take ? du : best; bi = take ? j : bi; bpos = take ? leaf * BVH_LEAF + t + u : bpos;
+        }
+    }
+}
+template <int DIM>
+__device__ __forceinline__ int leaf_eval(const BvhLeafT<DIM>* __restrict__ lf, int leaf, const f2* p2, float& best, int& bi, int& bpos, float& b2, int& l2, float& b3) {
+    const int prev_leaf = bpos >> 3; const float prev_best = best;
+    float dd[BVH_LEAF];
+    leaf_distances<DIM>(lf, p2, dd);
+    const float lo0 = fminf(fminf(dd[0], dd[1]), dd[2]), lo1 = fminf(fminf(dd[3], dd[4]), dd[5]), lo2 = fminf(dd[6], dd[7]);
+    const float m1 = fminf(fminf(lo0, lo1), lo2);
+    const float m = fminf(m1, FLT_MAX);
+    float x = m;
+    bool moved = false, scan = false;
+    int flags = 0;
+    if (m <= best) {
+        flags = 1;
+        bool e[BVH_LEAF];
+#pragma unroll
+        for (int t = 1; t < BVH_LEAF; t++) e[t] = dd[t] == m1;
+        const int ts = ((e[1] | e[3] | e[5] | e[7]) ? 1 : 0) | ((e[2] | e[3] | e[6] | e[7]) ? 2 : 0) | ((e[4] | e[5] | e[6] | e[7]) ? 4 : 0);
+        const int js = lf->idx[ts];
+        const float hi0 = __builtin_amdgcn_fmed3f(dd[0], dd[1], dd[2]), hi1 = __builtin_amdgcn_fmed3f(dd[3], dd[4], dd[5]), hi2 = __builtin_amdgcn_fmed3f(dd[6], dd[7], INFINITY);
+        const float lo01 = __builtin_amdgcn_fmed3f(lo0, lo1, -INFINITY), hi01 = __builtin_amdgcn_fmed3f(lo0, lo1, __builtin_amdgcn_fmed3f(hi0, hi1, -INFINITY));
+        const float m2 = __builtin_amdgcn_fmed3f(lo01, lo2, __builtin_amdgcn_fmed3f(hi01, hi2, -INFINITY));
+        const bool lt = m < best;
+        scan = !((m2 > m1) & (lt | (js == bi)));
+        if (!scan) {
+            x = __uint_as_float(min(__float_as_uint(m2), __float_as_uint(FLT_MAX)));
+            moved = lt & (prev_leaf != leaf);
+            best = lt ? m : best; bi = lt ? js : bi; bpos = lt ? leaf * BVH_LEAF + ts : bpos;
+        }
+    }
+    if (scan) {
+        flags = 3;
+        leaf_update_sequential<DIM>(lf, leaf, p2, prev_leaf == leaf, best, bi, bpos, x);
+        moved = prev_leaf != leaf && (bpos >> 3) == leaf;
+    }
+    others_insert(x, leaf, b2, l2, b3);
+    if (moved) others_insert(prev_best, prev_leaf, b2, l2, b3);
+    return flags;
 }
 
 template <int DIM>
@@ -406,9 +456,9 @@
 #pragma unroll
     for (int k = 0; k < DIM; k++) {
         const f2 lo0 = *(const f2*)&nd->lo[k][0], lo1 = *(const f2*)&nd->lo[k][2], hi0 = *(const f2*)&nd->hi[k][0], hi1 = *(const f2*)&nd->hi[k][2];
-        const f2 a0 = lo0 - p2[k], b0 = p2[k] - hi0, a1 = lo1 - p2[k], b1 = p2[k] - hi1;
-        const f2 e0 = {fmaxf(fmaxf(a0.x, b0.x), 0.f), fmaxf(fmaxf(a0.y, b0.y), 0.f)};
-        const f2 e1 = {fmaxf(fmaxf(a1.x, b1.x), 0.f), fmaxf(fmaxf(a1.y, b1.y), 0.f)};
+        const f2 c0 = {__builtin_amdgcn_fmed3f(p2[k].x, lo0.x, hi0.x), __builtin_amdgcn_fmed3f(p2[k].y, lo0.y, hi0.y)};
+        const f2 c1 = {__builtin_amdgcn_fmed3f(p2[k].x, lo1.x, hi1.x), __builtin_amdgcn_fmed3f(p2[k].y, lo1.y, hi1.y)};
+        const f2 e0 = p2[k] - c0, e1 = p2[k] - c1;
         const f2 s0 = e0 * e0, s1 = e1 * e1;
         l01 = (k == 0) ? s0 : l01 + s0;
         l23 = (k == 0) ? s1 : l23 + s1;
@@ -493,8 +543,10 @@
 #define ICP_DEBUG_WALK_TRACE 0
 #endif
 __device__ unsigned int g_walk_trace[64];
+#define WALK_BUDGET(i) do { if (lane == (int)__ffsll((long long)__ballot(true)) - 1) bud[i]++; } while (0)
 #else
 #define DEV_COUNT(i, n)
+#define WALK_BUDGET(i)
 #endif
 constexpr int XW_INTS = XW_CTRL + XW_SLOTS + XW_SLOTS * 5;
 constexpr int XW_SPIN_LIMIT = 1 << 22;
@@ -509,8 +561,12 @@
 
 template <int DIM, int NT, class MaskT, int MODE = 0>
 __device__ __forceinline__ void knn_walk_shared(const BvhViewT<DIM>& bv, float* p, float* keep3, bool need_walk, float& best, int& bi, int& bpos, float& lb_others, float& lb3, int& l2o,
-                                                uint2* __restrict__ lbq, int tid, int* fault = nullptr) {
+                                                uint2* __restrict__ lbq, int tid, int* fault = nullptr, int* budget = nullptr) {
     constexpr bool XW = MODE == 1 || MODE == 2, HELP = MODE == 2;
+#if ICP_DEBUG_TIMES
+    int bud[8] = {0, 0, 0, 0, 0, 0, 0, 0};
+#endif
+    (void)budget;
     static_assert(!XW || xw_enabled<DIM, NT>(), "cross-wave sharing: DIM 3, 2..8 waves per block");
     const int lane = tid & 63, Lq = bv.Lq, wbase = tid & ~63, myw = tid >> 6;
     uint2* R = lbq + wbase;
@@ -570,6 +626,7 @@
             const int n = act ? tbl[lane >> 2] : 0, j = lane & 3;
             f2 a01, a23;
             quad_lb_at<DIM>(bv, (0x55555555u & ((1u << (2 * L)) - 1u)) + (unsigned int)n, lq, a01, a23);
+            WALK_BUDGET(0);
             const float lbj = j == 0 ? a01.x : j == 1 ? a01.y : j == 2 ? a23.x : a23.y;
             const bool alive = act && !(lbj > thr_u);
             if (act && !alive) lmlb = min(lmlb, __float_as_uint(lbj));
@@ -600,8 +657,10 @@
             if (lane < nf) {
                 const int leaf = tbl[lane];
                 float xb = sb, x2 = FLT_MAX, x3 = FLT_MAX; int xi = si, xp = sp, xl = -1;
-                leaf_eval<DIM>(bv.leaves + leaf, leaf, lq.p2, xb, xi, xp, x2, xl, x3);
+                const int fl = leaf_eval<DIM>(bv.leaves + leaf, leaf, lq.p2, xb, xi, xp, x2, xl, x3); (void)fl;
+                WALK_BUDGET(1); if (fl & 1) WALK_BUDGET(2); if (fl & 2) WALK_BUDGET(3);
                 fold_part(wbase + wl, xb, xi, xp, x2, xl, x3, lmlb);
+                WALK_BUDGET(5);
             } else __hip_atomic_fetch_min((unsigned int*)(lbq + 6 * NT + wbase) + WAVE + wl, lmlb, __ATOMIC_RELAXED, __HIP_MEMORY_SCOPE_WORKGROUP);
             lone_done = true;
         }
@@ -611,7 +670,7 @@
     }
     QueryPt<DIM> qp;
     float wb; int wi, wp;
-    if constexpr (DIM == 3 && MODE == 1 && sizeof(MaskT) == 4) {
+    if constexpr (DIM == 3 && MODE == 1) {
         const uint2 ra_ = R[3 * NT + lane], rb_ = R[4 * NT + lane], rc_ = R[5 * NT + lane], rd_ = R[7 * NT + lane];
         float pq[3] = {__uint_as_float(rc_.y), __uint_as_float(rd_.x), __uint_as_float(rd_.y)};
         make_query<DIM>(bv, pq, qp);
@@ -626,12 +685,14 @@
             for (int L = 0; L < Lq; L++) {
                 f2 l01, l23;
                 quad_lb_at<DIM>(bv, (0x55555555u & ((1u << (2 * L)) - 1u)) + (unsigned int)idx, qp, l01, l23);
+                WALK_BUDGET(0);
                 const float m = fminf(fminf(l01.x, l01.y), fminf(l23.x, l23.y));
                 const int c = (l01.x == m) ? 0 : (l01.y == m) ? 1 : (l23.x == m) ? 2 : 3;
                 idx = (idx << 2) | c;
             }
             float u2 = FLT_MAX, u3 = FLT_MAX; int ul = -1;
-            leaf_eval<DIM>(bv.leaves + idx, idx, qp.p2, wb, wi, wp, u2, ul, u3);
+            const int fl = leaf_eval<DIM>(bv.leaves + idx, idx, qp.p2, wb, wi, wp, u2, ul, u3); (void)fl;
+            WALK_BUDGET(1); if (fl & 1) WALK_BUDGET(2); if (fl & 2) WALK_BUDGET(3);
         }
     }
     const unsigned long long wm = __ballot(need_walk);
@@ -648,12 +709,12 @@
     QuadStateT<MaskT> st; st.L = 0; st.idx = 0; st.pending = 0; st.alive = need_walk;
     float thr = fminf(wb * ICP_PRUNE_SLACK, FLT_MAX);
     auto descend = [&](const f2& l01, const f2& l23) {
-        const float m = fminf(fminf(l01.x, l01.y), fminf(l23.x, l23.y));
         const bool s0 = !(l01.x > thr), s1 = !(l01.y > thr), s2 = !(l23.x > thr), s3 = !(l23.y > thr);
         mlb = min(min(mlb, min(s0 ? NONE : __float_as_uint(l01.x), s1 ? NONE : __float_as_uint(l01.y))), min(s2 ? NONE : __float_as_uint(l23.x), s3 ? NONE : __float_as_uint(l23.y)));
-        if (!(m > thr)) {
-            const bool c0 = l01.x == m, c1 = l01.y == m, c2 = l23.x == m;
-            int c = 3; c = c2 ? 2 : c; c = c1 ? 1 : c; c = c0 ? 0 : c;
+        if (s0 | s1 | s2 | s3) {
+            const bool c01 = l01.y < l01.x, c23 = l23.y < l23.x;
+            const float m01 = c01 ? l01.y : l01.x, m23 = c23 ? l23.y : l23.x;
+            const int c = (m23 < m01) ? (c23 ? 3 : 2) : (c01 ? 1 : 0);
             const unsigned int pend = ((s0 ? 1u : 0u) | (s1 ? 2u : 0u) | (s2 ? 4u : 0u) | (s3 ? 8u : 0u)) & ~(1u << c);
             st.pending |= (MaskT)pend << (4 * st.L);
             st.idx = (st.idx << 2) | c; st.L++;
@@ -699,6 +760,7 @@
                 l01.x = (skip == 0 || skipB == 0) ? inf : l01.x; l01.y = (skip == 1 || skipB == 1) ? inf : l01.y;
                 l23.x = (skip == 2 || skipB == 2) ? inf : l23.x; l23.y = (skip == 3 || skipB == 3) ? inf : l23.y;
                 descend(l01, l23);
+                WALK_BUDGET(0);
             }
         }
         if (need_walk) { st.L = Lq; st.idx = wp >> 3; }
@@ -716,7 +778,9 @@
         trips++;
         if (tracer && trips < 56) g_walk_trace[7 + trips] = (unsigned int)wall_clock64();
 #endif
+        WALK_BUDGET(7);
         if (!st.alive && owner >= 0) {
+            WALK_BUDGET(5);
             fold_part(owner, wb, wi, wp, b2, l2, b3, mlb);
             if (XW && (owner >> 6) != myw) __hip_atomic_fetch_sub(xc + 4 + (owner >> 6), 1, __ATOMIC_RELEASE, __HIP_MEMORY_SCOPE_WORKGROUP);
             owner = -1;
@@ -728,6 +792,7 @@
             bool mine = false;
             if (sv == 1) { int expect = 1; mine = __hip_atomic_compare_exchange_strong(xstate + lane, &expect, 3, __ATOMIC_ACQUIRE, __ATOMIC_RELAXED, __HIP_MEMORY_SCOPE_WORKGROUP); }
             if (mine) {
+                WALK_BUDGET(6);
                 const uint2 ia = xa[lane], ib = xb[lane]; const int ip = xp[lane];
                 __hip_atomic_store(xstate + lane, 0, __ATOMIC_RELEASE, __HIP_MEMORY_SCOPE_WORKGROUP);
                 owner = (int)(ia.x & 0xFFFFu);
@@ -763,6 +828,7 @@
             const unsigned long long dm = __ballot(can);
             served = __popcll(im) <= __popcll(dm);
             if (!dm) break;
+            WALK_BUDGET(4);
             {
                 const int n = min(__popcll(im), __popcll(dm));
                 int* tbl = (int*)(R + 6 * NT);
@@ -799,6 +865,7 @@
             const bool can = st.alive && st.pending != 0;
             const unsigned long long dm = __ballot(can);
             if (dm) {
+                WALK_BUDGET(6);
                 const int sv = __hip_atomic_load(xstate + lane, __ATOMIC_RELAXED, __HIP_MEMORY_SCOPE_WORKGROUP);
                 const unsigned long long fm = __ballot(sv == 0);
                 const int n = min(__popcll(dm), __popcll(fm));
@@ -827,10 +894,12 @@
             f2 l01, l23;
             quad_lb_at<DIM>(bv, (0x55555555u & ((1u << (2 * st.L)) - 1u)) + (unsigned int)st.idx, qp, l01, l23);
             descend(l01, l23);
+            WALK_BUDGET(0);
             if (served ? __any(!st.alive) : __any(st.pending != 0)) break;
         }
         if (st.alive && st.L == Lq) {
-            leaf_eval<DIM>(bv.leaves + st.idx, st.idx, qp.p2, wb, wi, wp, b2, l2, b3);
+            const int fl = leaf_eval<DIM>(bv.leaves + st.idx, st.idx, qp.p2, wb, wi, wp, b2, l2, b3); (void)fl;
+            WALK_BUDGET(1); if (fl & 1) WALK_BUDGET(2); if (fl & 2) WALK_BUDGET(3);
             thr = fminf(wb * ICP_PRUNE_SLACK, FLT_MAX);
             st.alive = false;
             quad_pop_bits(st);
@@ -841,6 +910,16 @@
     if (tracer) { g_walk_trace[4] = (unsigned int)trips; g_walk_trace[5] = (unsigned int)polls; g_walk_trace[6] = (unsigned int)wall_clock64(); }
 #endif
     asm volatile("" ::"v"(0u));
+#if ICP_DEBUG_TIMES
+    if (budget) {
+#pragma unroll
+        for (int i = 0; i < 8; i++) {
+            int v = bud[i];
+            for (int o = 32; o > 0; o >>= 1) v += __shfl_xor(v, o, WAVE);
+            if (lane == 0 && v) atomicAdd(budget + i, v);
+        }
+    }
+#endif
     if (HELP) return;
     {
         const uint2 c = R[5 * NT + lane], d = R[7 * NT + lane], e = R[8 * NT + lane], f = R[9 * NT + lane];
@@ -868,11 +947,11 @@
 
 
 template <int DIM, int NT, class MaskT>
-__device__ __forceinline__ void xw_help(const BvhViewT<DIM>& bv, uint2* __restrict__ lbq, int tid, int* fault) {
+__device__ __forceinline__ void xw_help(const BvhViewT<DIM>& bv, uint2* __restrict__ lbq, int tid, int* fault, int* budget = nullptr) {
     float p[DIM], k3[3] = {0.f, 0.f, 0.f}, best = FLT_MAX, lbo = 0.f, lb3 = 0.f; int bi = -1, bpos = -1, l2 = -1;
 #pragma unroll
     for (int q = 0; q < DIM; q++) p[q] = 0.f;
-    knn_walk_shared<DIM, NT, MaskT, 2>(bv, p, k3, false, best, bi, bpos, lbo, lb3, l2, lbq, tid, fault);
+    knn_walk_shared<DIM, NT, MaskT, 2>(bv, p, k3, false, best, bi, bpos, lbo, lb3, l2, lbq, tid, fault, budget);
 }
 
 template <int DIM>
diff --git a/icp-variants_amd/csrc/dev_fused.hpp b/icp-variants_amd/csrc/dev_fused.hpp
--- a/icp-variants_amd/csrc/dev_fused.hpp
+++ b/icp-variants_amd/csrc/dev_fused.hpp
@@ -31,8 +31,10 @@
 #endif
 #if ICP_DEBUG_TIMES
 #define ICP_STAMP(j) do { if (kp.dbg_steps && lane == 0) kp.dbg_steps[8 * (wave_slot) + (j)] = (int)(unsigned int)wall_clock64(); } while (0)
+#define ICP_BUDGET_ROW(slot) ((kp.dbg_steps && 16 * kp.dbg_waves + 8 * 4096 <= kp.n) ? kp.dbg_steps + 8 * kp.dbg_waves + 8 * 4096 + 8 * (slot) : nullptr)
 #else
 #define ICP_STAMP(j)
+#define ICP_BUDGET_ROW(slot) nullptr
 #endif
 
 template <int DIM> struct QueryIn {
@@ -146,8 +148,16 @@
         for (int q = 0; q < DIM; q++) { p2[q].x = p[q]; p2[q].y = p[q]; }
         float b2 = FLT_MAX, b3 = FLT_MAX; int nl2 = -1;
         const int lf = q0 >> 3;
-        leaf_eval<DIM>(bv.leaves + lf, lf, p2, best, bi, bpos, b2, nl2, b3);
-        if (l2 >= 0 && l2 != lf) leaf_eval<DIM>(bv.leaves + l2, l2, p2, best, bi, bpos, b2, nl2, b3);
+        if constexpr (DIM == 3) {
+#pragma unroll 1
+            for (int r = 0; r < 2; r++) {
+                const int lx = r ? l2 : lf;
+                if (r == 0 || (l2 >= 0 && l2 != lf)) leaf_eval<DIM>(bv.leaves + lx, lx, p2, best, bi, bpos, b2, nl2, b3);
+            }
+        } else {
+            leaf_eval<DIM>(bv.leaves + lf, lf, p2, best, bi, bpos, b2, nl2, b3);
+            if (l2 >= 0 && l2 != lf) leaf_eval<DIM>(bv.leaves + l2, l2, p2, best, bi, bpos, b2, nl2, b3);
+        }
         lb_others = fminf(sqrt_dn(b2), lb3);
         lb3 = fminf(sqrt_dn(b3), lb3);
         l2 = nl2;
@@ -156,11 +166,14 @@
 #if ICP_DEBUG_STEPS && !ICP_DEBUG_TIMES
     if (k >= 0 && kp.dbg_steps) kp.dbg_steps[k] = need_walk ? -1 : two_leaf ? -2 : 0;
 #endif
+#if ICP_DEBUG_TIMES
+    if (int* row = ICP_BUDGET_ROW(wave_slot)) { if (lane < 8) row[lane] = 0; }
+#endif
     bool walked = false;
     if (__any(need_walk)) {
         walked = true;
         float rn[3] = {rn0, rn1, rn2};
-        knn_walk_shared<DIM, BVH_THREADS, typename std::conditional<WIDE, unsigned long long, unsigned int>::type, XW ? 1 : 0>(bv, p, rn, need_walk, best, bi, bpos, lb_others, lb3, l2, bvh_lbq, tid, kp.fault);
+        knn_walk_shared<DIM, BVH_THREADS, typename std::conditional<WIDE, unsigned long long, unsigned int>::type, XW ? 1 : 0>(bv, p, rn, need_walk, best, bi, bpos, lb_others, lb3, l2, bvh_lbq, tid, kp.fault, ICP_BUDGET_ROW(wave_slot));
         rn0 = rn[0]; rn1 = rn[1]; rn2 = rn[2];
         q0 = -2;
         fused_front_clear<DIM>(in);
@@ -267,7 +280,7 @@
             bvh_lbq[3 * NT + tid] = make_uint2(__float_as_uint(o.s0), __float_as_uint(o.s1)); bvh_lbq[4 * NT + tid] = make_uint2(__float_as_uint(o.s2), __float_as_uint(o.d0));
             bvh_lbq[5 * NT + tid] = make_uint2(__float_as_uint(o.d1), __float_as_uint(o.d2)); bvh_lbq[7 * NT + tid] = make_uint2(__float_as_uint(o.n0), __float_as_uint(o.n1));
             bvh_lbq[8 * NT + tid] = make_uint2(__float_as_uint(o.n2), __float_as_uint(o.wt)); bvh_lbq[9 * NT + tid] = make_uint2(o.valid ? 1u : 0u, 0u);
-            xw_help<DIM, NT, typename std::conditional<WIDE, unsigned long long, unsigned int>::type>(bv, bvh_lbq, tid, kp.fault);
+            xw_help<DIM, NT, typename std::conditional<WIDE, unsigned long long, unsigned int>::type>(bv, bvh_lbq, tid, kp.fault, ICP_BUDGET_ROW(wave_slot));
             const uint2 a = bvh_lbq[3 * NT + tid], b = bvh_lbq[4 * NT + tid], c = bvh_lbq[5 * NT + tid], d = bvh_lbq[7 * NT + tid], e = bvh_lbq[8 * NT + tid], f = bvh_lbq[9 * NT + tid];
             o.s0 = __uint_as_float(a.x); o.s1 = __uint_as_float(a.y); o.s2 = __uint_as_float(b.x); o.d0 = __uint_as_float(b.y); o.d1 = __uint_as_float(c.x); o.d2 = __uint_as_float(c.y);
             o.n0 = __uint_as_float(d.x); o.n1 = __uint_as_float(d.y); o.n2 = __uint_as_float(e.x); o.wt = __uint_as_float(e.y); o.valid = f.x != 0u;
diff --git a/icp-variants_amd/csrc/host_debug.hpp b/icp-variants_amd/csrc/host_debug.hpp
--- a/icp-variants_amd/csrc/host_debug.hpp
+++ b/icp-variants_amd/csrc/host_debug.hpp
@@ -77,6 +77,63 @@
     return ICP_OK;
 }
 
+__global__ void k_debug_walk_steps(int n_leaves, const icpdev::BvhLeafT<3>* leaves, const float* lq, const int* leaf_no, const float* sf, const int* si, float* of, int* oi,
+                                   int n_nodes, const icpdev::BvhQuadT<3>* nodes, const float* nq, float* bounds) {
+    const int i = blockIdx.x * blockDim.x + threadIdx.x;
+    if (i < n_leaves) {
+        icpdev::f2 p2[3];
+        for (int k = 0; k < 3; k++) { p2[k].x = lq[3 * i + k]; p2[k].y = p2[k].x; }
+        float best = sf[3 * i], b2 = sf[3 * i + 1], b3 = sf[3 * i + 2]; int bi = si[3 * i], bpos = si[3 * i + 1], l2 = si[3 * i + 2];
+        const int flags = icpdev::leaf_eval<3>(leaves + i, leaf_no[i], p2, best, bi, bpos, b2, l2, b3);
+        of[3 * i] = best; of[3 * i + 1] = b2; of[3 * i + 2] = b3; oi[4 * i] = bi; oi[4 * i + 1] = bpos; oi[4 * i + 2] = l2; oi[4 * i + 3] = flags;
+    }
+    if (i < n_nodes) {
+        icpdev::f2 p2[3], l01, l23;
+        for (int k = 0; k < 3; k++) { p2[k].x = nq[3 * i + k]; p2[k].y = p2[k].x; }
+        icpdev::quad_lb<3>(nodes + i, p2, l01, l23);
+        bounds[4 * i] = l01.x; bounds[4 * i + 1] = l01.y; bounds[4 * i + 2] = l23.x; bounds[4 * i + 3] = l23.y;
+    }
+}
+int icp_debug_walk_steps(icp_ctx* c, int32_t n_leaves, const void* leaves, const float* lq, const int32_t* leaf_no, const float* sf, const int32_t* si, float* of, int32_t* oi,
+                         int32_t n_nodes, const void* nodes, const float* nq, float* bounds, float* empty_box) {
+    if (!c || n_leaves < 0 || n_nodes < 0 || n_leaves > (1 << 20) || n_nodes > (1 << 20)) return ICP_ERR_INVALID_ARG;
+    if (n_leaves > 0 && (!leaves || !lq || !leaf_no || !sf || !si || !of || !oi)) return ICP_ERR_INVALID_ARG;
+    if (n_nodes > 0 && (!nodes || !nq || !bounds)) return ICP_ERR_INVALID_ARG;
+    if (empty_box) { empty_box[0] = icpdev::BVH_QUAD_EMPTY_LO; empty_box[1] = icpdev::BVH_QUAD_EMPTY_HI; }
+    const int n = n_leaves > n_nodes ? n_leaves : n_nodes;
+    if (n == 0) return ICP_OK;
+    int rc;
+    if ((rc = set_device(c))) return rc;
+    DrainOnError guard(c);
+    const size_t L = (size_t)n_leaves, N = (size_t)n_nodes;
+    auto up = [](size_t x) { return (x + 127) & ~(size_t)127; };
+    const size_t o_lq = 128 * L, o_no = up(o_lq + 12 * L), o_sf = up(o_no + 4 * L), o_si = up(o_sf + 12 * L), o_nd = up(o_si + 12 * L), o_nq = o_nd + 128 * N, o_of = up(o_nq + 12 * N),
+                 o_oi = up(o_of + 12 * L), o_bd = up(o_oi + 16 * L), total = o_bd + 16 * N;
+    if ((rc = ensure(c, c->staging, total))) return rc;
+    char* d = c->staging.as<char>();
+    if (L) {
+        HIPCK(c, hipMemcpyAsync(d, leaves, 128 * L, hipMemcpyHostToDevice, c->stream));
+        HIPCK(c, hipMemcpyAsync(d + o_lq, lq, 12 * L, hipMemcpyHostToDevice, c->stream));
+        HIPCK(c, hipMemcpyAsync(d + o_no, leaf_no, 4 * L, hipMemcpyHostToDevice, c->stream));
+        HIPCK(c, hipMemcpyAsync(d + o_sf, sf, 12 * L, hipMemcpyHostToDevice, c->stream));
+        HIPCK(c, hipMemcpyAsync(d + o_si, si, 12 * L, hipMemcpyHostToDevice, c->stream));
+    }
+    if (N) {
+        HIPCK(c, hipMemcpyAsync(d + o_nd, nodes, 128 * N, hipMemcpyHostToDevice, c->stream));
+        HIPCK(c, hipMemcpyAsync(d + o_nq, nq, 12 * N, hipMemcpyHostToDevice, c->stream));
+    }
+    hipLaunchKernelGGL(k_debug_walk_steps, dim3((unsigned)((n + 255) / 256)), dim3(256), 0, c->stream, n_leaves, (const icpdev::BvhLeafT<3>*)d, (const float*)(d + o_lq), (const int*)(d + o_no),
+                       (const float*)(d + o_sf), (const int*)(d + o_si), (float*)(d + o_of), (int*)(d + o_oi), n_nodes, (const icpdev::BvhQuadT<3>*)(d + o_nd), (const float*)(d + o_nq), (float*)(d + o_bd));
+    HIPCK(c, hipGetLastError());
+    if (L) {
+        HIPCK(c, hipMemcpyAsync(of, d + o_of, 12 * L, hipMemcpyDeviceToHost, c->stream));
+        HIPCK(c, hipMemcpyAsync(oi, d + o_oi, 16 * L, hipMemcpyDeviceToHost, c->stream));
+    }
+    if (N) HIPCK(c, hipMemcpyAsync(bounds, d + o_bd, 16 * N, hipMemcpyDeviceToHost, c->stream));
+    HIPCK(c, hipStreamSynchronize(c->stream));
+    return guard.done();
+}
+
 int icp_selftest_wave_reduce(icp_ctx* c, const double* in, double* out, int32_t* lane_of) {
     if (!c || !in || !out || !lane_of) return ICP_ERR_INVALID_ARG;
     int rc;
```

Result: faster. 35240, median of 6 (+3.6%).
